# OpenPPL/ppq

Hardware: AMD Instinct MI355X
Metric: calibration samples/sec (RuntimeCalibrationPass, KL 2048-bin, ResNet-50 INT8) (higher is better)
Workload: dtype f32; 1 GPU; ResNet-50 topology (53 Conv + 1 Gemm, BN folded, seeded He init), RuntimeCalibrationPass kl 2048 bins, per-tensor INT8 activations, per-channel INT8 weights, 279 batches x 32 x 3x224x224 per GPU; samples=8928, batch=32, observed_tensors=72, rccl_ranks=1, async_observe=False, cache_params=False, channels_last=False, fuse_params=True, batch_observations=True, reuse_activations=False, replayed_batches=0, hip_graph=auto, graph_replays=0, miopen_find=False

## Files before the change

### include/ppq_hip.h

```cpp
#ifndef PPQ_HIP_H_
#define PPQ_HIP_H_

#include <stdint.h>

#ifdef __cplusplus
extern "C" {
#endif

typedef enum {
    PPQHIP_OK = 0,
    PPQHIP_ERR_INVALID_VALUE = -1,
    PPQHIP_ERR_UNSUPPORTED = -2,
    PPQHIP_ERR_HIP = -3
} ppqhip_status;

#define PPQHIP_ABI_VERSION 4

const char* ppqhip_last_error(void);
int ppqhip_version(void);
int ppqhip_device_arch(char* buf, int n);

int ppqhip_fq_linear_t(const float* x, const float* scale, const float* offset, float* out,
                       int64_t n, int clip_min, int clip_max, int rounding, void* stream);

int ppqhip_fq_linear_c(const float* x, const float* scale, const float* offset, float* out,
                       int64_t n, int64_t num_channel, int64_t elem_per_channel,
                       int clip_min, int clip_max, int rounding, void* stream);

int ppqhip_to_int_t(const float* x, const float* scale, const float* offset, void* out, int64_t n,
                    int clip_min, int clip_max, int rounding, int out_dtype, void* stream);
int ppqhip_to_int_c(const float* x, const float* scale, const float* offset, void* out, int64_t n,
                    int64_t num_channel, int64_t elem_per_channel, int clip_min, int clip_max,
                    int rounding, int out_dtype, void* stream);

typedef struct ppqhip_fq_job {
    const float* x;
    const float* scale;
    const float* offset;
    float* out;
    int64_t n, num_channel, elem_per_channel;
    int32_t clip_min, clip_max;
} ppqhip_fq_job;
int64_t ppqhip_fq_linear_multi_table_bytes(int num_jobs);
int ppqhip_fq_linear_multi(const ppqhip_fq_job* jobs, int num_jobs, int rounding, void* device_table,
                           int upload, void* stream);

int ppqhip_fq_linear_t_bwd(const float* x, const float* scale, const float* offset,
                           const float* grad_y, float* grad_x, float* grad_s, int64_t n,
                           int clip_min, int clip_max, int rounding, void* stream);

int ppqhip_fq_linear_c_bwd(const float* x, const float* scale, const float* offset,
                           const float* grad_y, float* grad_x, float* grad_s, int64_t n,
                           int64_t num_channel, int64_t elem_per_channel,
                           int clip_min, int clip_max, int rounding, void* stream);

int64_t ppqhip_fq_linear_t_bwd_partials(int64_t n);
int ppqhip_fq_linear_t_bwd_main(const float* x, const float* scale, const float* offset, const float* grad_y, float* grad_x,
                                float* partial, int64_t n, int clip_min, int clip_max, int rounding, void* stream);
typedef struct ppqhip_lsq_finish_job {
    const float* partial;
    float* grad_s;
    int64_t n;
    int32_t clip_min, clip_max;
} ppqhip_lsq_finish_job;
int ppqhip_lsq_finish_multi(const ppqhip_lsq_finish_job* jobs, int num_jobs, void* stream);

typedef struct ppqhip_lsq_job {
    const float* x;
    const float* scale;
    const float* offset;
    const float* grad_y;
    float* grad_x;
    float* grad_s;
    int64_t n, num_channel, elem_per_channel;
    int32_t clip_min, clip_max;
} ppqhip_lsq_job;
int ppqhip_fq_linear_c_bwd_multi(const ppqhip_lsq_job* jobs, int num_jobs, int rounding, void* stream);

int ppqhip_fq_float_t(const float* x, const float* scale, const float* offset, float* out,
                      int64_t n, int exponent, int mantissa, float clip_min, float clip_max,
                      int rounding, void* stream);

int ppqhip_fq_float_c(const float* x, const float* scale, const float* offset, float* out,
                      int64_t n, int64_t num_channel, int64_t elem_per_channel,
                      int exponent, int mantissa, float clip_min, float clip_max,
                      int rounding, void* stream);

typedef struct ppqhip_float_search_job {
    const float* x;
    int64_t rows, row_len;
    int32_t exponent, mantissa;
    float clip_min, clip_max;
} ppqhip_float_search_job;
int64_t ppqhip_float_scale_search_table_bytes(int num_jobs);
int ppqhip_float_scale_search(const ppqhip_float_search_job* jobs, int num_jobs, const float* candidates,
                              int num_candidates, int rounding, void* device_table, double* out, void* stream);

typedef struct ppqhip_fq_float_job {
    const float* x;
    const float* scale;
    const float* offset;
    float* out;
    int64_t n, num_channel, elem_per_channel;
    int32_t exponent, mantissa;
    float clip_min, clip_max;
} ppqhip_fq_float_job;
int64_t ppqhip_fq_float_multi_table_bytes(int num_jobs);
int ppqhip_fq_float_multi(const ppqhip_fq_float_job* jobs, int num_jobs, int rounding, void* device_table,
                          int upload, void* stream);

int ppqhip_fq_float_c_bwd(const float* x, const float* scale, const float* offset,
                          const float* grad_y, float* grad_x, float* grad_s, int64_t n,
                          int64_t num_channel, int64_t elem_per_channel,
                          int exponent, int mantissa, float clip_min, float clip_max,
                          int rounding, void* stream);

int64_t ppqhip_hist_workspace_bytes(int64_t n, int64_t num_bins);
int ppqhip_hist_sym_t(const float* x, int64_t n, float hist_scale, int clip_outliers,
                      int32_t* hist, int64_t num_bins, void* workspace, void* stream);

int ppqhip_hist_asym_t(const float* x, int64_t n, float min_value, float max_value,
                       int clip_outliers, int32_t* hist, int64_t num_bins, void* workspace,
                       void* stream);

int ppqhip_hist_sym_c(const float* x, int64_t n, int64_t num_channel, int64_t elem_per_channel,
                      float hist_scale, int clip_outliers, int32_t* hist, int64_t num_bins,
                      void* stream);

int ppqhip_hist_sym_c_scales(const float* x, int64_t n, int64_t num_channel, int64_t elem_per_channel,
                             const float* hist_scales, int clip_outliers, int32_t* hist,
                             int64_t num_bins, void* stream);
int ppqhip_hist_asym_c_ranges(const float* x, int64_t n, int64_t num_channel, int64_t elem_per_channel,
                              const float* mins, const float* maxs, int clip_outliers, int32_t* hist,
                              int64_t num_bins, void* stream);

int64_t ppqhip_quantile_workspace_bytes(int64_t n);
int ppqhip_quantile_t(const float* x, int64_t n, float q, float* dest, uint32_t* hint, void* workspace,
                      void* stream);

typedef struct ppqhip_quantile_job {
    const float* x;
    float* dest;
    uint32_t* hint;
    int64_t n;
} ppqhip_quantile_job;
int64_t ppqhip_quantile_multi_workspace_bytes(int num_jobs, int64_t total_elems);
int ppqhip_quantile_t_multi(const ppqhip_quantile_job* jobs, int num_jobs, float q, void* workspace,
                            void* stream);
void ppqhip_quantile_debug_layout(int64_t* out);
void ppqhip_quantile_hot_layout(int64_t* out);

int ppqhip_isotone_t(const float* x, int64_t n, float* dest, void* workspace, void* stream);

int64_t ppqhip_minmax_workspace_bytes(int64_t n);
int ppqhip_minmax_t(const float* x, int64_t n, float* minmax, void* workspace, void* stream);

int ppqhip_minmax_c(const float* x, int64_t n, int64_t num_channel, int64_t elem_per_channel,
                    float* mins, float* maxs, void* stream);

typedef struct ppqhip_minmax_c_job {
    const float* x;
    float* mins;
    float* maxs;
    int64_t n, num_channel, elem_per_channel;
    int32_t fresh, reserved;
} ppqhip_minmax_c_job;
int ppqhip_minmax_c_multi(const ppqhip_minmax_c_job* jobs, int num_jobs, void* stream);

int ppqhip_channel_sum(const float* x, int64_t n, int64_t num_channel, int64_t elem_per_channel,
                       double* sums, void* stream);

int64_t ppqhip_hist_rows(void);
int ppqhip_hist_sym_t_rows(const float* x, int64_t n, float hist_scale, int clip_outliers,
                           int32_t* rows, int64_t num_bins, void* stream);
int ppqhip_hist_asym_t_rows(const float* x, int64_t n, float min_value, float max_value,
                            int clip_outliers, int32_t* rows, int64_t num_bins, void* stream);
typedef struct ppqhip_minmax_job {
    const float* x;
    float* slots;
    int64_t n;
} ppqhip_minmax_job;
int ppqhip_minmax_t_slots_multi(const ppqhip_minmax_job* jobs, int num_jobs, void* stream);

typedef struct ppqhip_hist_job {
    const float* x;
    int32_t* rows;
    int64_t n;
    float p0, p1;
} ppqhip_hist_job;
int ppqhip_hist_t_rows_multi(const ppqhip_hist_job* jobs, int num_jobs, int asymmetric,
                             int clip_outliers, int64_t num_bins, void* stream);
int ppqhip_hist_rows_finish(const int32_t* rows, int64_t num_bins, int32_t* hist, void* stream);
int ppqhip_check_bin_rule(const float* x, int64_t n, float min_value, float hist_scale, int asymmetric, uint64_t* out, void* stream);
int64_t ppqhip_minmax_slots(void);
int ppqhip_minmax_t_slots(const float* x, int64_t n, float* slots, void* stream);
int ppqhip_minmax_slots_finish(const float* slots, float* minmax, void* stream);

float ppqhip_mse_loss_host(const int64_t* hist, int64_t num_bins, int start, int step, int end);

int64_t ppqhip_mse_search_workspace_bytes(int64_t num_hist);
int ppqhip_mse_search(const int32_t* hist, int64_t num_hist, int64_t num_bins,
                      const double* hist_scale, const double* min_value,
                      int quant_min, int quant_max, int symmetrical, int32_t* best,
                      void* workspace, void* stream);

int64_t ppqhip_kl_num_candidates(int64_t num_bins, int num_of_bits);
int ppqhip_kl_losses(const int32_t* hist, int64_t num_hist, int64_t num_bins, int num_of_bits,
                     double* losses, void* stream);

int ppqhip_tensor_clip_t(const float* value, const float* reference, const float* limit,
                         float* out, int64_t n, void* stream);
int ppqhip_tensor_clip_c(const float* value, const float* reference, const float* limit,
                         float* out, int64_t n, int64_t num_channel, int64_t elem_per_channel,
                         void* stream);
int ppqhip_rounding_loss(const float* x, const float* scale, const float* offset, float* out,
                         int64_t n, int64_t num_channel, int64_t elem_per_channel,
                         int clip_min, int clip_max, int rounding, void* stream);
int ppqhip_rounding_loss_bwd(const float* x, const float* dy, const float* scale,
                             const float* offset, float* dx, int64_t n, int64_t num_channel,
                             int64_t elem_per_channel, int clip_min, int clip_max, int rounding,
                             void* stream);

int ppqhip_bias_act(float* y, const float* bias, int64_t n, int64_t num_channel, int64_t elem_per_channel,
                    int relu, void* stream);
int ppqhip_bias_add_act(float* a, const float* bias_a, float* b, const float* bias_b, float* out,
                        int64_t n, int64_t num_channel, int64_t elem_per_channel, int relu, void* stream);

typedef struct ppqhip_adaround_job {
    const float* w;
    const float* v;
    const float* scale;
    const float* offset;
    float* out;
    const float* dy;
    int64_t n, num_channel, elem_per_channel;
    int32_t qmin, qmax;
} ppqhip_adaround_job;
int ppqhip_adaround_fwd_multi(const ppqhip_adaround_job* jobs, int num_jobs, void* stream);
int ppqhip_adaround_bwd_multi(const ppqhip_adaround_job* jobs, int num_jobs, const float* reg, void* stream);

typedef struct ppqhip_roundtune_job {
    const float* w;
    const float* r;
    const float* scale;
    const float* offset;
    float* out;
    int64_t n, num_channel, elem_per_channel;
    int32_t qmin, qmax;
} ppqhip_roundtune_job;
int ppqhip_roundtune_fwd_multi(const ppqhip_roundtune_job* jobs, int num_jobs, void* stream);

typedef struct ppqhip_fetch_rows_job {
    const float* x;
    const int32_t* index;
    float* out;
    int64_t rows, row_len, count;
} ppqhip_fetch_rows_job;
int ppqhip_fetch_rows_multi(const ppqhip_fetch_rows_job* jobs, int num_jobs, void* stream);
typedef struct ppqhip_measure_rows_job {
    const float* p;
    const float* r;
    const int32_t* index;
    double* sums;
    int64_t rows, row_len, count;
} ppqhip_measure_rows_job;
int ppqhip_measure_rows_multi(const ppqhip_measure_rows_job* jobs, int num_jobs, void* stream);
enum { PPQHIP_MEASURE_SNR = 0, PPQHIP_MEASURE_MSE = 1, PPQHIP_MEASURE_COSINE = 2 };
enum { PPQHIP_REDUCE_MEAN = 0, PPQHIP_REDUCE_MAX = 1 };
typedef struct ppqhip_measure_finish_job {
    const double* sums;
    double* acc;
    float* row_out;
    int64_t rows, count;
    int32_t method, reduce;
} ppqhip_measure_finish_job;
int ppqhip_measure_finish_multi(const ppqhip_measure_finish_job* jobs, int num_jobs, void* stream);

typedef struct ppqhip_equalize_segment {
    const float* base;
    int64_t extent;
    int64_t div, a, b;
    int64_t outer, stride, run;
    float multiplier;
    int32_t downstream;
} ppqhip_equalize_segment;
typedef struct ppqhip_equalize_scale_job {
    const ppqhip_equalize_segment* segments;
    float* scale;
    int32_t num_segments, num_channel;
    float value_threshold;
    int32_t reserved;
} ppqhip_equalize_scale_job;
int ppqhip_equalize_scale_multi(const ppqhip_equalize_scale_job* jobs, int num_jobs, void* stream);
typedef struct ppqhip_equalize_apply_job {
    float* x;
    const float* scale;
    int64_t n, run, inner, group_out;
    int64_t num_scale;
    int32_t divide, reserved;
} ppqhip_equalize_apply_job;
int ppqhip_equalize_apply_multi(const ppqhip_equalize_apply_job* jobs, int num_jobs, void* stream);

typedef struct ppqhip_split_plan_job {
    const ppqhip_equalize_segment* segments;
    int32_t* src_of;
    int32_t* count;
    int32_t num_segments, num_channel;
    float value_threshold;
    int32_t reserved;
} ppqhip_split_plan_job;
int ppqhip_split_plan_multi(const ppqhip_split_plan_job* jobs, int num_jobs, void* stream);
typedef struct ppqhip_split_apply_job {
    const float* x;
    float* out;
    const int32_t* src_of;
    int64_t n, run;
    int32_t num_channel, count;
} ppqhip_split_apply_job;
int ppqhip_split_apply_multi(const ppqhip_split_apply_job* jobs, int num_jobs, void* stream);

typedef struct ppqhip_ssd_scales_job {
    ppqhip_equalize_segment first, last;
    const float* act_range;
    float* scales;
    float* ranges;
    int32_t num_channel;
    float channel_ratio;
} ppqhip_ssd_scales_job;
int ppqhip_ssd_scales_multi(const ppqhip_ssd_scales_job* jobs, int num_jobs, void* stream);
typedef struct ppqhip_ssd_apply_job {
    const float* x;
    float* out;
    const float* scales;
    int64_t n, run, inner, group_out;
    int64_t num_channel;
    int32_t divide, reserved;
} ppqhip_ssd_apply_job;
int ppqhip_ssd_apply_multi(const ppqhip_ssd_apply_job* jobs, int num_jobs, void* stream);
typedef struct ppqhip_fq_measure_rows_job {
    const float* y;
    const float* r;
    const float* scale;
    const float* offset;
    double* sums;
    int64_t rows, count;
    int64_t num_channel, elem_per_channel;
    int32_t clip_min, clip_max, rounding, reserved;
} ppqhip_fq_measure_rows_job;
int ppqhip_fq_measure_rows_multi(const ppqhip_fq_measure_rows_job* jobs, int num_jobs, void* stream);

typedef struct ppqhip_stat_job {
    const float* p;
    const float* r;
    float* rec;
    int64_t n;
    int32_t bins, reserved;
} ppqhip_stat_job;
int ppqhip_stat_moments_multi(const ppqhip_stat_job* jobs, int num_jobs, void* stream);
int ppqhip_stat_shape_multi(const ppqhip_stat_job* jobs, int num_jobs, void* stream);

enum { PPQHIP_MXFP8_E4M3 = 0, PPQHIP_MXFP8_E5M2 = 1, PPQHIP_MXFP6_E3M2 = 2, PPQHIP_MXFP6_E2M3 = 3, PPQHIP_MXFP4_E2M1 = 4,
       PPQHIP_MXINT8 = 5 };
int ppqhip_mx_fq(const float* x, float* y, uint8_t* scale_codes, int64_t outer, int64_t axis_len, int64_t inner, int format,
                 void* stream);
typedef struct ppqhip_mx_job {
    const float* x;
    float* y;
    uint8_t* scale_codes;
    int64_t outer, axis_len, inner;
    int32_t format, reserved;
} ppqhip_mx_job;
int ppqhip_mx_fq_multi(const ppqhip_mx_job* jobs, int num_jobs, void* stream);

int ppqhip_mx_pack(const float* x, uint8_t* elements, uint8_t* scales, int64_t outer, int64_t axis_len, int64_t inner, int format,
                   void* stream);
typedef struct ppqhip_mx_pack_job {
    const float* x;
    uint8_t* elements;
    uint8_t* scales;
    int64_t outer, axis_len, inner;
    int32_t format, reserved;
} ppqhip_mx_pack_job;
int ppqhip_mx_pack_multi(const ppqhip_mx_pack_job* jobs, int num_jobs, void* stream);
int ppqhip_mx_unpack(const uint8_t* elements, const uint8_t* scales, float* y, int64_t outer, int64_t axis_len, int64_t inner,
                     int format, void* stream);
typedef struct ppqhip_mx_unpack_job {
    const uint8_t* elements;
    const uint8_t* scales;
    float* y;
    int64_t outer, axis_len, inner;
    int32_t format, reserved;
} ppqhip_mx_unpack_job;
int ppqhip_mx_unpack_multi(const ppqhip_mx_unpack_job* jobs, int num_jobs, void* stream);

int ppqhip_mx_gemm(const uint8_t* a_elements, const uint8_t* a_scales, int a_format, const uint8_t* b_elements,
                   const uint8_t* b_scales, int b_format, const float* bias, float* c, int64_t m, int64_t n, int64_t k,
                   void* stream);

int ppqhip_mx_conv2d(const uint8_t* x_elements, const uint8_t* x_scales, int x_format, const uint8_t* w_elements,
                     const uint8_t* w_scales, int w_format, const float* bias, float* y, int64_t n, int64_t c, int64_t h, int64_t w,
                     int64_t o, int64_t kh, int64_t kw, int64_t stride_h, int64_t stride_w, int64_t pad_h, int64_t pad_w,
                     int64_t dil_h, int64_t dil_w, void* stream);

#define PPQHIP_PROF_MAX_KERNELS 48
typedef struct {
    char name[48];
    int64_t launches;
    double total_ms;
    double total_bytes;
} ppqhip_prof_entry;
int ppqhip_prof_enable(int on);
int ppqhip_prof_collect(ppqhip_prof_entry* entries, int max_entries);
double ppqhip_prof_event_overhead_us(void* stream, int pairs);

#ifdef __cplusplus
}
#endif
#endif
```

### ppq_amd/_lib.py

```python
import ctypes
import os

_HERE = os.path.dirname(os.path.abspath(__file__))
LIB_PATH = os.path.join(_HERE, 'libppq_hip.so')

c_f32p = ctypes.c_void_p
c_i32p = ctypes.c_void_p
c_f64p = ctypes.c_void_p
c_i64 = ctypes.c_int64
c_int = ctypes.c_int
c_flt = ctypes.c_float
c_vp = ctypes.c_void_p

ABI_VERSION = 4


class ProfEntry(ctypes.Structure):
    _fields_ = [('name', ctypes.c_char * 48), ('launches', ctypes.c_int64),
                ('total_ms', ctypes.c_double), ('total_bytes', ctypes.c_double)]


PROTOTYPES = {
    'ppqhip_last_error': (ctypes.c_char_p, []),
    'ppqhip_version': (c_int, []),
    'ppqhip_device_arch': (c_int, [ctypes.c_char_p, c_int]),
    'ppqhip_fq_linear_t': (c_int, [c_f32p, c_f32p, c_f32p, c_f32p, c_i64, c_int, c_int, c_int, c_vp]),
    'ppqhip_fq_linear_c': (c_int, [c_f32p, c_f32p, c_f32p, c_f32p, c_i64, c_i64, c_i64, c_int, c_int, c_int, c_vp]),
    'ppqhip_to_int_t': (c_int, [c_f32p, c_f32p, c_f32p, c_vp, c_i64, c_int, c_int, c_int, c_int, c_vp]),
    'ppqhip_to_int_c': (c_int, [c_f32p, c_f32p, c_f32p, c_vp, c_i64, c_i64, c_i64, c_int, c_int, c_int, c_int, c_vp]),
    'ppqhip_fq_linear_t_bwd': (c_int, [c_f32p, c_f32p, c_f32p, c_f32p, c_f32p, c_f32p, c_i64, c_int, c_int, c_int,
                                       c_vp]),
    'ppqhip_fq_linear_c_bwd': (c_int, [c_f32p, c_f32p, c_f32p, c_f32p, c_f32p, c_f32p, c_i64, c_i64, c_i64, c_int,
                                       c_int, c_int, c_vp]),
    'ppqhip_fq_linear_c_bwd_multi': (c_int, [c_vp, c_int, c_int, c_vp]),
    'ppqhip_fq_linear_t_bwd_partials': (c_i64, [c_i64]),
    'ppqhip_fq_linear_t_bwd_main': (c_int, [c_f32p, c_f32p, c_f32p, c_f32p, c_f32p, c_f32p, c_i64, c_int, c_int, c_int, c_vp]),
    'ppqhip_lsq_finish_multi': (c_int, [c_vp, c_int, c_vp]),
    'ppqhip_bias_act': (c_int, [c_f32p, c_f32p, c_i64, c_i64, c_i64, c_int, c_vp]),
    'ppqhip_bias_add_act': (c_int, [c_f32p, c_f32p, c_f32p, c_f32p, c_f32p, c_i64, c_i64, c_i64, c_int, c_vp]),
    'ppqhip_fq_float_t': (c_int, [c_f32p, c_f32p, c_f32p, c_f32p, c_i64, c_int, c_int, c_flt, c_flt, c_int, c_vp]),
    'ppqhip_fq_float_c': (c_int, [c_f32p, c_f32p, c_f32p, c_f32p, c_i64, c_i64, c_i64, c_int, c_int, c_flt, c_flt,
                                  c_int, c_vp]),
    'ppqhip_fq_float_c_bwd': (c_int, [c_f32p, c_f32p, c_f32p, c_f32p, c_f32p, c_f32p, c_i64, c_i64, c_i64, c_int,
                                      c_int, c_flt, c_flt, c_int, c_vp]),
    'ppqhip_hist_workspace_bytes': (c_i64, [c_i64, c_i64]),
    'ppqhip_hist_sym_t': (c_int, [c_f32p, c_i64, c_flt, c_int, c_i32p, c_i64, c_vp, c_vp]),
    'ppqhip_hist_asym_t': (c_int, [c_f32p, c_i64, c_flt, c_flt, c_int, c_i32p, c_i64, c_vp, c_vp]),
    'ppqhip_hist_sym_c': (c_int, [c_f32p, c_i64, c_i64, c_i64, c_flt, c_int, c_i32p, c_i64, c_vp]),
    'ppqhip_hist_sym_c_scales': (c_int, [c_f32p, c_i64, c_i64, c_i64, c_f32p, c_int, c_i32p, c_i64, c_vp]),
    'ppqhip_hist_asym_c_ranges': (c_int, [c_f32p, c_i64, c_i64, c_i64, c_f32p, c_f32p, c_int, c_i32p, c_i64, c_vp]),
    'ppqhip_quantile_workspace_bytes': (c_i64, [c_i64]),
    'ppqhip_quantile_t': (c_int, [c_f32p, c_i64, c_flt, c_f32p, c_vp, c_vp, c_vp]),
    'ppqhip_isotone_t': (c_int, [c_f32p, c_i64, c_f32p, c_vp, c_vp]),
    'ppqhip_minmax_workspace_bytes': (c_i64, [c_i64]),
    'ppqhip_minmax_t': (c_int, [c_f32p, c_i64, c_f32p, c_vp, c_vp]),
    'ppqhip_minmax_c': (c_int, [c_f32p, c_i64, c_i64, c_i64, c_f32p, c_f32p, c_vp]),
    'ppqhip_minmax_c_multi': (c_int, [c_vp, c_int, c_vp]),
    'ppqhip_fq_linear_multi_table_bytes': (c_i64, [c_int]),
    'ppqhip_fq_linear_multi': (c_int, [c_vp, c_int, c_int, c_vp, c_int, c_vp]),
    'ppqhip_float_scale_search_table_bytes': (c_i64, [c_int]),
    'ppqhip_float_scale_search': (c_int, [c_vp, c_int, c_vp, c_int, c_int, c_vp, c_vp, c_vp]),
    'ppqhip_fq_float_multi_table_bytes': (c_i64, [c_int]),
    'ppqhip_fq_float_multi': (c_int, [c_vp, c_int, c_int, c_vp, c_int, c_vp]),
    'ppqhip_quantile_multi_workspace_bytes': (c_i64, [c_int, c_i64]),
    'ppqhip_quantile_t_multi': (c_int, [c_vp, c_int, c_flt, c_vp, c_vp]),
    'ppqhip_quantile_debug_layout': (None, [c_vp]),
    'ppqhip_quantile_hot_layout': (None, [c_vp]),
    'ppqhip_minmax_t_slots_multi': (c_int, [c_vp, c_int, c_vp]),
    'ppqhip_hist_t_rows_multi': (c_int, [c_vp, c_int, c_int, c_int, c_i64, c_vp]),
    'ppqhip_channel_sum': (c_int, [c_f32p, c_i64, c_i64, c_i64, c_f64p, c_vp]),
    'ppqhip_hist_rows': (c_i64, []),
    'ppqhip_hist_sym_t_rows': (c_int, [c_f32p, c_i64, c_flt, c_int, c_i32p, c_i64, c_vp]),
    'ppqhip_hist_asym_t_rows': (c_int, [c_f32p, c_i64, c_flt, c_flt, c_int, c_i32p, c_i64, c_vp]),
    'ppqhip_hist_rows_finish': (c_int, [c_i32p, c_i64, c_i32p, c_vp]),
    'ppqhip_check_bin_rule': (c_int, [c_f32p, c_i64, c_flt, c_flt, c_int, c_vp, c_vp]),
    'ppqhip_minmax_slots': (c_i64, []),
    'ppqhip_minmax_t_slots': (c_int, [c_f32p, c_i64, c_f32p, c_vp]),
    'ppqhip_minmax_slots_finish': (c_int, [c_f32p, c_f32p, c_vp]),
    'ppqhip_mse_loss_host': (c_flt, [ctypes.POINTER(ctypes.c_int64), c_i64, c_int, c_int, c_int]),
    'ppqhip_mse_search_workspace_bytes': (c_i64, [c_i64]),
    'ppqhip_mse_search': (c_int, [c_i32p, c_i64, c_i64, c_f64p, c_f64p, c_int, c_int, c_int, c_i32p, c_vp, c_vp]),
    'ppqhip_kl_num_candidates': (c_i64, [c_i64, c_int]),
    'ppqhip_kl_losses': (c_int, [c_i32p, c_i64, c_i64, c_int, c_f64p, c_vp]),
    'ppqhip_tensor_clip_t': (c_int, [c_f32p, c_f32p, c_f32p, c_f32p, c_i64, c_vp]),
    'ppqhip_tensor_clip_c': (c_int, [c_f32p, c_f32p, c_f32p, c_f32p, c_i64, c_i64, c_i64, c_vp]),
    'ppqhip_rounding_loss': (c_int, [c_f32p, c_f32p, c_f32p, c_f32p, c_i64, c_i64, c_i64, c_int, c_int, c_int, c_vp]),
    'ppqhip_rounding_loss_bwd': (c_int, [c_f32p, c_f32p, c_f32p, c_f32p, c_f32p, c_i64, c_i64, c_i64, c_int, c_int,
                                         c_int, c_vp]),
    'ppqhip_adaround_fwd_multi': (c_int, [c_vp, c_int, c_vp]),
    'ppqhip_adaround_bwd_multi': (c_int, [c_vp, c_int, c_f32p, c_vp]),
    'ppqhip_roundtune_fwd_multi': (c_int, [c_vp, c_int, c_vp]),
    'ppqhip_equalize_scale_multi': (c_int, [c_vp, c_int, c_vp]),
    'ppqhip_equalize_apply_multi': (c_int, [c_vp, c_int, c_vp]),
    'ppqhip_split_plan_multi': (c_int, [c_vp, c_int, c_vp]),
    'ppqhip_split_apply_multi': (c_int, [c_vp, c_int, c_vp]),
    'ppqhip_ssd_scales_multi': (c_int, [c_vp, c_int, c_vp]),
    'ppqhip_ssd_apply_multi': (c_int, [c_vp, c_int, c_vp]),
    'ppqhip_fq_measure_rows_multi': (c_int, [c_vp, c_int, c_vp]),
    'ppqhip_fetch_rows_multi': (c_int, [c_vp, c_int, c_vp]),
    'ppqhip_measure_rows_multi': (c_int, [c_vp, c_int, c_vp]),
    'ppqhip_measure_finish_multi': (c_int, [c_vp, c_int, c_vp]),
    'ppqhip_stat_moments_multi': (c_int, [c_vp, c_int, c_vp]),
    'ppqhip_stat_shape_multi': (c_int, [c_vp, c_int, c_vp]),
    'ppqhip_mx_fq': (c_int, [c_f32p, c_f32p, c_vp, c_i64, c_i64, c_i64, c_int, c_vp]),
    'ppqhip_mx_fq_multi': (c_int, [c_vp, c_int, c_vp]),
    'ppqhip_mx_pack': (c_int, [c_f32p, c_vp, c_vp, c_i64, c_i64, c_i64, c_int, c_vp]),
    'ppqhip_mx_pack_multi': (c_int, [c_vp, c_int, c_vp]),
    'ppqhip_mx_unpack': (c_int, [c_vp, c_vp, c_f32p, c_i64, c_i64, c_i64, c_int, c_vp]),
    'ppqhip_mx_unpack_multi': (c_int, [c_vp, c_int, c_vp]),
    'ppqhip_mx_gemm': (c_int, [c_vp, c_vp, c_int, c_vp, c_vp, c_int, c_f32p, c_f32p, c_i64, c_i64, c_i64, c_vp]),
    'ppqhip_prof_enable': (c_int, [c_int]),
    'ppqhip_mx_conv2d': (c_int, [c_vp, c_vp, c_int, c_vp, c_vp, c_int, c_f32p, c_f32p] + [c_i64] * 13 + [c_vp]),
    'ppqhip_prof_collect': (c_int, [ctypes.POINTER(ProfEntry), c_int]),
    'ppqhip_prof_event_overhead_us': (ctypes.c_double, [c_vp, c_int]),
}

if not os.path.exists(LIB_PATH):
    raise ImportError(
        f'{LIB_PATH} is missing: the HIP kernel library has not been built.  Run '
        '`python -c "import __graft_entry__ as g; g.build()"` or `make -C ppq_amd/csrc` (needs hipcc, '
        'targets gfx950).  ppq_amd has no CPU / PyTorch fallback by design.')

import torch

_torch_hip = os.path.join(os.path.dirname(torch.__file__), 'lib', 'libamdhip64.so')
if os.path.exists(_torch_hip):
    ctypes.CDLL(_torch_hip, mode=ctypes.RTLD_GLOBAL)

try:
    lib = ctypes.CDLL(LIB_PATH)
except OSError as e:
    raise ImportError(f'cannot load {LIB_PATH}: {e}') from e

for _name, (_res, _args) in PROTOTYPES.items():
    _fn = getattr(lib, _name)
    _fn.restype = _res
    _fn.argtypes = _args


if lib.ppqhip_version() != ABI_VERSION:
    raise ImportError(f'{LIB_PATH} has ABI version {lib.ppqhip_version()}, this package needs {ABI_VERSION}: rebuild it '
                      '(`make -C ppq_amd/csrc` or `python -c "import __graft_entry__ as g; g.build()"`)')


def last_error() -> str:
    msg = lib.ppqhip_last_error()
    return msg.decode('utf-8', 'replace') if msg else ''
```

### ppq_amd/csrc/epilogue.hip

```cpp
#include "common.hpp"

namespace ppqhip {
namespace {

constexpr int kEpTileU = 2;
constexpr int kEpSmallU = 1;
constexpr long long kEpSmallElems = 1ll << 20;

struct EpArgs {
    float* a;
    const float* bias_a;
    float* b;
    const float* bias_b;
    float* out;
    uint32_t nvec;
    uint32_t tail;
    int ntail;
    FastDiv epc;
    FastDiv nc;
};

__device__ __forceinline__ uint32_t channel_of(uint32_t i, const FastDiv& epc, const FastDiv& nc) {
    const uint32_t row = fdiv(i, epc);
    return row - fdiv(row, nc) * nc.d;
}

__device__ __forceinline__ float act(float v, bool relu) {
    return (relu && !__builtin_isnan(v)) ? __builtin_fmaxf(v, 0.f) : v;
}

__device__ __forceinline__ float4 add4(const float4& x, const float4& y) {
    return make_float4(x.x + y.x, x.y + y.y, x.z + y.z, x.w + y.w);
}

template <bool RELU>
__device__ __forceinline__ float4 act4(const float4& v) {
    return make_float4(act(v.x, RELU), act(v.y, RELU), act(v.z, RELU), act(v.w, RELU));
}

template <bool PLANE>
__device__ __forceinline__ float4 bias4(const float* __restrict__ bias, uint32_t v, const FastDiv& epc, const FastDiv& nc) {
    if (PLANE) {
        const float t = bias[channel_of(v, epc, nc)];
        return make_float4(t, t, t, t);
    }
    const uint32_t i = v * 4u;
    return make_float4(bias[channel_of(i, epc, nc)], bias[channel_of(i + 1, epc, nc)], bias[channel_of(i + 2, epc, nc)],
                       bias[channel_of(i + 3, epc, nc)]);
}

template <bool RESID, bool BIAS_B, bool RELU>
__device__ __forceinline__ void epilogue_elem(const EpArgs& p, uint32_t i, const FastDiv& epc) {
    const uint32_t c = channel_of(i, epc, p.nc);
    const float x = p.a[i] + p.bias_a[c];
    if (!RESID) { p.a[i] = act(x, RELU); return; }
    p.a[i] = x;
    float y = p.b[i];
    if (BIAS_B) { y = y + p.bias_b[c]; p.b[i] = y; }
    p.out[i] = act(x + y, RELU);
}

template <int U, bool RESID, bool BIAS_B, bool RELU, bool PLANE>
__global__ __launch_bounds__(kBlock) void epilogue_kernel(EpArgs p) {
    const uint32_t base = blockIdx.x * (kBlock * U) + threadIdx.x;
    float4* a4 = reinterpret_cast<float4*>(p.a);
    float4* b4 = reinterpret_cast<float4*>(p.b);
    float4* o4 = reinterpret_cast<float4*>(p.out);
    float4 a[U], ba[U], b[U], bb[U];
#pragma unroll
    for (int k = 0; k < U; k++) {
        const uint32_t vv = min(base + k * kBlock, p.nvec - 1);
        a[k] = a4[vv];
        ba[k] = bias4<PLANE>(p.bias_a, vv, p.epc, p.nc);
        if (RESID) b[k] = b4[vv];
        if (BIAS_B) bb[k] = bias4<PLANE>(p.bias_b, vv, p.epc, p.nc);
    }
#pragma unroll
    for (int k = 0; k < U; k++) {
        const uint32_t vv = base + k * kBlock;
        if (vv >= p.nvec) continue;
        const float4 x = add4(a[k], ba[k]);
        if (!RESID) { a4[vv] = act4<RELU>(x); continue; }
        a4[vv] = x;
        float4 y = b[k];
        if (BIAS_B) { y = add4(y, bb[k]); b4[vv] = y; }
        o4[vv] = act4<RELU>(add4(x, y));
    }
    if (!PLANE && blockIdx.x == 0 && (int)threadIdx.x < p.ntail)
        epilogue_elem<RESID, BIAS_B, RELU>(p, p.tail + threadIdx.x, p.epc);
}

template <bool RESID, bool BIAS_B, bool RELU>
__global__ __launch_bounds__(kBlock) void epilogue_scalar_kernel(EpArgs p) {
    const uint32_t stride = gridDim.x * kBlock;
    for (uint32_t i = blockIdx.x * kBlock + threadIdx.x; i < (uint32_t)p.ntail; i += stride)
        epilogue_elem<RESID, BIAS_B, RELU>(p, i, p.epc);
}

template <bool RESID, bool BIAS_B, bool RELU>
void launch_epilogue(EpArgs p, int64_t n, int64_t C, int64_t epc, bool aligned, hipStream_t st) {
    p.nc = make_fastdiv((uint32_t)C);
    if (!aligned || n < 4) {
        p.nvec = 0; p.tail = 0; p.ntail = (int)n;
        p.epc = make_fastdiv((uint32_t)epc);
        hipLaunchKernelGGL((epilogue_scalar_kernel<RESID, BIAS_B, RELU>), dim3(stream_grid(n, kBlock)), dim3(kBlock), 0, st, p);
        return;
    }
    p.nvec = (uint32_t)(n >> 2);
    p.tail = p.nvec * 4u;
    p.ntail = (int)(n & 3);
    const bool plane = (epc % 4 == 0);
    p.epc = make_fastdiv((uint32_t)(plane ? epc / 4 : epc));
#define PPQ_LAUNCH_EP(U, PLANE)                                                                                          \
    hipLaunchKernelGGL((epilogue_kernel<U, RESID, BIAS_B, RELU, PLANE>), dim3((p.nvec + kBlock * U - 1) / (kBlock * U)),   \
                       dim3(kBlock), 0, st, p)
    if (n <= kEpSmallElems) {
        if (plane) PPQ_LAUNCH_EP(kEpSmallU, true); else PPQ_LAUNCH_EP(kEpSmallU, false);
    } else {
        if (plane) PPQ_LAUNCH_EP(kEpTileU, true); else PPQ_LAUNCH_EP(kEpTileU, false);
    }
#undef PPQ_LAUNCH_EP
}

int validate(int64_t n, int64_t C, int64_t epc, const char* what) {
    if (n <= 0 || n > 0x7fffffffLL) {
        set_error("%s: n=%lld is empty or has more than 2^31 - 1 elements", what, (long long)n);
        return PPQHIP_ERR_INVALID_VALUE;
    }
    if (C <= 0 || epc <= 0 || C > 0x7fffffffLL || epc > 0x7fffffffLL || n % (C * epc) != 0) {
        set_error("%s: n=%lld is not [outer, %lld channels, %lld elem/channel]", what, (long long)n, (long long)C,
                  (long long)epc);
        return PPQHIP_ERR_INVALID_VALUE;
    }
    return PPQHIP_OK;
}

}
}

using namespace ppqhip;

extern "C" {

int ppqhip_bias_act(float* y, const float* bias, int64_t n, int64_t num_channel, int64_t elem_per_channel, int relu,
                    void* stream) {
    if (int st = validate(n, num_channel, elem_per_channel, "bias_act")) return st;
    if (!y || !bias) { set_error("bias_act: null pointer"); return PPQHIP_ERR_INVALID_VALUE; }
    hipStream_t s = (hipStream_t)stream;
    EpArgs p{};
    p.a = y; p.bias_a = bias;
    const bool aligned = aligned16(y);
    if (relu) launch_epilogue<false, false, true>(p, n, num_channel, elem_per_channel, aligned, s);
    else launch_epilogue<false, false, false>(p, n, num_channel, elem_per_channel, aligned, s);
    return finish_launch("bias_act");
}

int ppqhip_bias_add_act(float* a, const float* bias_a, float* b, const float* bias_b, float* out, int64_t n,
                        int64_t num_channel, int64_t elem_per_channel, int relu, void* stream) {
    if (int st = validate(n, num_channel, elem_per_channel, "bias_add_act")) return st;
    if (!a || !bias_a || !b || !out) { set_error("bias_add_act: null pointer"); return PPQHIP_ERR_INVALID_VALUE; }
    hipStream_t s = (hipStream_t)stream;
    EpArgs p{};
    p.a = a; p.bias_a = bias_a; p.b = b; p.bias_b = bias_b; p.out = out;
    const bool aligned = aligned16(a) && aligned16(b) && aligned16(out);
    if (bias_b) {
        if (relu) launch_epilogue<true, true, true>(p, n, num_channel, elem_per_channel, aligned, s);
        else launch_epilogue<true, true, false>(p, n, num_channel, elem_per_channel, aligned, s);
    } else {
        if (relu) launch_epilogue<true, false, true>(p, n, num_channel, elem_per_channel, aligned, s);
        else launch_epilogue<true, false, false>(p, n, num_channel, elem_per_channel, aligned, s);
    }
    return finish_launch("bias_add_act");
}

}
```

### ppq_amd/csrc/reduce.hip

```cpp
#include <cmath>
#include <cstdlib>
#include <vector>

#include "common.hpp"

namespace ppqhip {

__device__ __forceinline__ void block_minmax_commit(float mn, float mx, float* gmin, float* gmax, float* lds) {
    mn = wave_min(mn);
    mx = wave_max(mx);
    const int wid = threadIdx.x >> 6, lane = threadIdx.x & 63, nw = blockDim.x >> 6;
    if (lane == 0) { lds[wid] = mn; lds[8 + wid] = mx; }
    __syncthreads();
    if (threadIdx.x == 0) {
        for (int w = 1; w < nw; w++) { mn = fminf(mn, lds[w]); mx = fmaxf(mx, lds[8 + w]); }
        if (mn <= mx) {
            atomic_min_f32(gmin, mn);
            atomic_max_f32(gmax, mx);
        }
    }
}

template <int U, bool NT>
__global__ __launch_bounds__(kBlock) void minmax_t_kernel(const float* __restrict__ x, uint32_t n, int vec_ok,
                                                          float* __restrict__ minmax, float* __restrict__ partial,
                                                          int accumulate) {
    __shared__ float lds[16];
    float mn = INFINITY, mx = -INFINITY;
    stream_elems<U, NT>(x, n, vec_ok != 0, [&](float a) { mn = fminf(mn, a); mx = fmaxf(mx, a); });
    if (partial == nullptr) { block_minmax_commit(mn, mx, &minmax[0], &minmax[1], lds); return; }
    mn = wave_min(mn);
    mx = wave_max(mx);
    const int wid = threadIdx.x >> 6, lane = threadIdx.x & 63;
    if (lane == 0) { lds[wid] = mn; lds[8 + wid] = mx; }
    __syncthreads();
    if (threadIdx.x == 0) {
        for (int w = 1; w < kBlock / kWave; w++) { mn = fminf(mn, lds[w]); mx = fmaxf(mx, lds[8 + w]); }
        if (accumulate) {
            mn = fminf(mn, partial[2 * blockIdx.x]);
            mx = fmaxf(mx, partial[2 * blockIdx.x + 1]);
        }
        partial[2 * blockIdx.x] = mn;
        partial[2 * blockIdx.x + 1] = mx;
    }
}

constexpr int kMinMaxMultiMax = 96;
constexpr int kMMBlock = 256, kMMU = 2;
constexpr int kMMWgPerCu = 8;
constexpr int kMMGrid = kNumCU * kMMWgPerCu;
constexpr uint32_t kMMTileVec = (uint32_t)kMMBlock * kMMU, kMMTileElems = kMMTileVec * 4;
static_assert(kMMGrid <= kNumCU * 8, "one slot per workgroup");
struct MinMaxJob {
    const float* x;
    float* slots;
    uint32_t n;
    uint32_t first_tile;
};
struct MinMaxJobs {
    MinMaxJob job[kMinMaxMultiMax];
    uint32_t count;
    uint32_t total_tiles;
};
__host__ __device__ inline uint32_t mm_job_tiles(uint32_t n, bool vec_ok) {
    if (!vec_ok) return (n + kMMTileElems - 1) / kMMTileElems;
    const uint32_t full = (n >> 2) / kMMTileVec;
    return full + (n > full * kMMTileElems ? 1u : 0u);
}

template <bool NT>
__global__ __launch_bounds__(kMMBlock) void minmax_persistent_kernel(const MinMaxJobs jobs) {
    __shared__ float lds[32];
    const uint32_t G = gridDim.x, g = blockIdx.x;
    uint32_t t, t_end;
    even_split(jobs.total_tiles, G, g, t, t_end);
    if (t >= t_end) return;
    uint32_t lo = 0, hi = jobs.count;
    while (hi - lo > 1) {
        const uint32_t mid = (lo + hi) >> 1;
        if (jobs.job[mid].first_tile <= t) lo = mid; else hi = mid;
    }
    for (uint32_t j = lo; t < t_end; j++) {
        const MinMaxJob& job = jobs.job[j];
        const uint32_t j_end = (j + 1 < jobs.count) ? jobs.job[j + 1].first_tile : jobs.total_tiles;
        uint32_t k = t - job.first_tile;
        const uint32_t k1 = min(t_end, j_end) - job.first_tile;
        t = min(t_end, j_end);
        const float* __restrict__ x = job.x;
        const uint32_t n = job.n;
        const bool vec_ok = (reinterpret_cast<uintptr_t>(x) & 15u) == 0;
        const uint32_t full = vec_ok ? (n >> 2) / kMMTileVec : 0u;
        const uint32_t kf = min(k1, full);
        float mn = INFINITY, mx = -INFINITY;
        if (k < kf) {
            const float4* xv = reinterpret_cast<const float4*>(x) + threadIdx.x;
            float4 bufa[kMMU], bufb[kMMU];
            auto fetch = [&](float4 (&buf)[kMMU], uint32_t tile) {
                const float4* p = xv + (size_t)tile * kMMTileVec;
#pragma unroll
                for (int u = 0; u < kMMU; u++) buf[u] = load4<NT>(p + u * kMMBlock);
            };
            auto consume = [&](const float4 (&buf)[kMMU]) {
#pragma unroll
                for (int u = 0; u < kMMU; u++) {
                    mn = fminf(fminf(mn, buf[u].x), fminf(buf[u].y, fminf(buf[u].z, buf[u].w)));
                    mx = fmaxf(fmaxf(mx, buf[u].x), fmaxf(buf[u].y, fmaxf(buf[u].z, buf[u].w)));
                }
            };
            fetch(bufa, k);
            for (;;) {
                fetch(bufb, min(k + 1, kf - 1));
                consume(bufa);
                if (++k >= kf) break;
                fetch(bufa, min(k + 1, kf - 1));
                consume(bufb);
                if (++k >= kf) break;
            }
        }
        for (; k < k1; k++) {
            const uint32_t e0 = k * kMMTileElems + threadIdx.x;
#pragma unroll 4
            for (int r = 0; r < 4 * kMMU; r++) {
                const uint32_t i = e0 + r * kMMBlock;
                if (i < n) { const float a = x[i]; mn = fminf(mn, a); mx = fmaxf(mx, a); }
            }
        }
        mn = wave_min(mn);
        mx = wave_max(mx);
        const int wid = threadIdx.x >> 6, lane = threadIdx.x & 63;
        if (lane == 0) { lds[wid] = mn; lds[16 + wid] = mx; }
        __syncthreads();
        if (threadIdx.x == 0) {
            for (int w = 1; w < kMMBlock / kWave; w++) { mn = fminf(mn, lds[w]); mx = fmaxf(mx, lds[16 + w]); }
            job.slots[2 * g] = fminf(mn, job.slots[2 * g]);
            job.slots[2 * g + 1] = fmaxf(mx, job.slots[2 * g + 1]);
        }
        __syncthreads();
    }
}

template <int K, bool PING = false, bool NT = false>
__global__ __launch_bounds__(kMMBlock) void minmax_small_kernel(const float* __restrict__ x, uint32_t n, float* __restrict__ slots) {
    __shared__ float lds[32];
    const uint32_t G = gridDim.x, g = blockIdx.x;
    float s_mn = INFINITY, s_mx = -INFINITY;
    if (threadIdx.x == 0) { s_mn = slots[2 * g]; s_mx = slots[2 * g + 1]; }
    const uint32_t nvec = n >> 2, full_rows = nvec / kMMBlock;
    uint32_t r0, r1;
    even_split(full_rows, G, g, r0, r1);
    const float4* xv = reinterpret_cast<const float4*>(x) + threadIdx.x;
    float mn = INFINITY, mx = -INFINITY;
    auto fetch = [&](float4 (&buf)[K], uint32_t r) {
#pragma unroll
        for (int k = 0; k < K; k++) buf[k] = load4<NT>(xv + (size_t)min(r + (uint32_t)k, r1 - 1) * kMMBlock);
    };
    auto fold = [&](const float4 (&buf)[K]) {
#pragma unroll
        for (int k = 0; k < K; k++) {
            mn = fminf(fminf(mn, buf[k].x), fminf(buf[k].y, fminf(buf[k].z, buf[k].w)));
            mx = fmaxf(fmaxf(mx, buf[k].x), fmaxf(buf[k].y, fmaxf(buf[k].z, buf[k].w)));
        }
    };
    if (PING) {
        if (r0 < r1) {
            float4 bufa[K], bufb[K];
            uint32_t r = r0;
            fetch(bufa, r);
            for (;;) {
                fetch(bufb, r + K);
                fold(bufa);
                r += K;
                if (r >= r1) break;
                fetch(bufa, r + K);
                fold(bufb);
                r += K;
                if (r >= r1) break;
            }
        }
    } else {
        for (uint32_t r = r0; r < r1; r += K) {
            float4 buf[K];
            fetch(buf, r);
            fold(buf);
        }
    }
    if (g == G - 1) {
        for (uint32_t i = full_rows * kMMBlock * 4 + threadIdx.x; i < n; i += kMMBlock) { const float a = x[i]; mn = fminf(mn, a); mx = fmaxf(mx, a); }
    }
    mn = wave_min(mn);
    mx = wave_max(mx);
    const int wid = threadIdx.x >> 6, lane = threadIdx.x & 63;
    if (lane == 0) { lds[wid] = mn; lds[16 + wid] = mx; }
    __syncthreads();
    if (threadIdx.x == 0) {
        for (int w = 1; w < kMMBlock / kWave; w++) { mn = fminf(mn, lds[w]); mx = fmaxf(mx, lds[16 + w]); }
        slots[2 * g] = fminf(mn, s_mn);
        slots[2 * g + 1] = fmaxf(mx, s_mx);
    }
}

__global__ __launch_bounds__(kBlock) void minmax_finish_kernel(const float* __restrict__ partial, uint32_t count,
                                                               float* __restrict__ minmax) {
    __shared__ float lds[16];
    float mn = INFINITY, mx = -INFINITY;
    for (uint32_t i = threadIdx.x; i < count; i += kBlock) {
        mn = fminf(mn, partial[2 * i]);
        mx = fmaxf(mx, partial[2 * i + 1]);
    }
    mn = wave_min(mn);
    mx = wave_max(mx);
    const int wid = threadIdx.x >> 6, lane = threadIdx.x & 63;
    if (lane == 0) { lds[wid] = mn; lds[8 + wid] = mx; }
    __syncthreads();
    if (threadIdx.x == 0) {
        for (int w = 1; w < kBlock / kWave; w++) { mn = fminf(mn, lds[w]); mx = fmaxf(mx, lds[8 + w]); }
        minmax[0] = fminf(minmax[0], mn);
        minmax[1] = fmaxf(minmax[1], mx);
    }
}

constexpr int kMMCU = 16;
constexpr int kMMCWavesPerCu = 16;
constexpr uint32_t kMMCChunk = 8192;
__global__ __launch_bounds__(kBlock) void minmax_c_wave_kernel(const float* __restrict__ x, uint32_t epc, int vec_ok, uint32_t C,
                                                               uint32_t outer, uint32_t K, uint32_t chunks, uint32_t items,
                                                               float* __restrict__ mins, float* __restrict__ maxs) {
    const uint32_t item = blockIdx.x * (kBlock / kWave) + (threadIdx.x >> 6);
    if (item >= items) return;
    const uint32_t lane = threadIdx.x & 63;
    const uint32_t rc = item / chunks, chunk = item - rc * chunks;
    const uint32_t g = rc / C, c = rc - g * C;
    const uint32_t n0 = g * K, n1 = min(n0 + K, outer);
    const uint32_t lo = chunk * kMMCChunk, hi = min(lo + kMMCChunk, epc);
    float mn = INFINITY, mx = -INFINITY;
    for (uint32_t n = n0; n < n1; n++) {
        const float* xr = x + ((size_t)n * C + c) * epc;
        if (vec_ok) {
            const float4* xv = reinterpret_cast<const float4*>(xr);
            const uint32_t v1 = hi >> 2;
            for (uint32_t v0 = (lo >> 2) + lane; v0 < v1; v0 += 64 * kMMCU) {
                float4 a[kMMCU];
#pragma unroll
                for (int u = 0; u < kMMCU; u++) a[u] = xv[min(v0 + 64 * u, v1 - 1)];
#pragma unroll
                for (int u = 0; u < kMMCU; u++) {
                    mn = fminf(fminf(mn, a[u].x), fminf(a[u].y, fminf(a[u].z, a[u].w)));
                    mx = fmaxf(fmaxf(mx, a[u].x), fmaxf(a[u].y, fmaxf(a[u].z, a[u].w)));
                }
            }
        } else {
            for (uint32_t j = lo + lane; j < hi; j += 64) { const float a = xr[j]; mn = fminf(mn, a); mx = fmaxf(mx, a); }
        }
    }
    mn = wave_min(mn);
    mx = wave_max(mx);
    if (lane == 0 && mn <= mx) { atomic_min_f32(&mins[c], mn); atomic_max_f32(&maxs[c], mx); }
}

__global__ __launch_bounds__(kBlock) void minmax_c_generic_kernel(const float* __restrict__ x, uint32_t n,
                                                                  FastDiv elem_per_channel, FastDiv num_channel,
                                                                  int use_lds, float* __restrict__ mins,
                                                                  float* __restrict__ maxs) {
    extern __shared__ float mm[];
    const uint32_t C = num_channel.d;
    if (use_lds) {
        for (uint32_t c = threadIdx.x; c < C; c += kBlock) { mm[c] = INFINITY; mm[C + c] = -INFINITY; }
        __syncthreads();
    }
    const uint32_t stride = gridDim.x * kBlock;
    for (uint32_t i = blockIdx.x * kBlock + threadIdx.x; i < n; i += stride) {
        const float a = x[i];
        if (a != a) continue;
        const uint32_t row = fdiv(i, elem_per_channel);
        const uint32_t c = row - fdiv(row, num_channel) * C;
        if (use_lds) { atomic_min_f32(&mm[c], a); atomic_max_f32(&mm[C + c], a); }
        else { atomic_min_f32(&mins[c], a); atomic_max_f32(&maxs[c], a); }
    }
    if (use_lds) {
        __syncthreads();
        for (uint32_t c = threadIdx.x; c < C; c += kBlock) {
            if (mm[c] <= mm[C + c]) { atomic_min_f32(&mins[c], mm[c]); atomic_max_f32(&maxs[c], mm[C + c]); }
        }
    }
}

__device__ __forceinline__ double wave_sum_f64(double v) {
#pragma unroll
    for (int m = 32; m > 0; m >>= 1) v += __shfl_xor(v, m, 64);
    return v;
}

__global__ __launch_bounds__(kBlock) void channel_sum_row_kernel(const float* __restrict__ x, uint32_t rows_per_channel,
                                                                 uint32_t C, uint32_t epc, int vec_ok,
                                                                 double* __restrict__ partial) {
    __shared__ double lds[kBlock / kWave];
    const uint32_t c = blockIdx.x, s = blockIdx.y, S = gridDim.y;
    double acc = 0.0;
    for (uint32_t n = s; n < rows_per_channel; n += S) {
        const float* xr = x + ((size_t)n * C + c) * epc;
        if (vec_ok) {
            const float4* xv = reinterpret_cast<const float4*>(xr);
            const uint32_t v1 = epc >> 2;
            for (uint32_t v = threadIdx.x; v < v1; v += 4 * kBlock) {
                float4 a[4];
#pragma unroll
                for (int u = 0; u < 4; u++) a[u] = xv[min(v + u * kBlock, v1 - 1)];
#pragma unroll
                for (int u = 0; u < 4; u++)
                    if (v + u * kBlock < v1) acc += ((double)a[u].x + (double)a[u].y) + ((double)a[u].z + (double)a[u].w);
            }
        } else {
            for (uint32_t j = threadIdx.x; j < epc; j += kBlock) acc += (double)xr[j];
        }
    }
    acc = wave_sum_f64(acc);
    const int wid = threadIdx.x >> 6, lane = threadIdx.x & 63;
    if (lane == 0) lds[wid] = acc;
    __syncthreads();
    if (threadIdx.x == 0) {
        double t = lds[0];
        for (int w = 1; w < kBlock / kWave; w++) t += lds[w];
        partial[(size_t)s * C + c] = t;
    }
}

__global__ __launch_bounds__(kBlock) void channel_sum_single_kernel(const float* __restrict__ x, uint32_t rows_per_channel, uint32_t C,
                                                                    uint32_t epc, double* __restrict__ sums) {
    __shared__ double lds[kBlock / kWave];
    const uint32_t c = blockIdx.x;
    const uint32_t v1 = epc >> 2;
    double acc = 0.0;
    const double seed = threadIdx.x == 0 ? sums[c] : 0.0;
    for (uint32_t n = 0; n < rows_per_channel; n += 2) {
        const float4* x0 = reinterpret_cast<const float4*>(x + ((size_t)n * C + c) * epc);
        const float4* x1 = reinterpret_cast<const float4*>(x + ((size_t)min(n + 1, rows_per_channel - 1) * C + c) * epc);
        const bool two = n + 1 < rows_per_channel;
        for (uint32_t v = threadIdx.x; v < v1; v += 4 * kBlock) {
            float4 a[4], b[4];
#pragma unroll
            for (int u = 0; u < 4; u++) { a[u] = x0[min(v + u * kBlock, v1 - 1)]; b[u] = x1[min(v + u * kBlock, v1 - 1)]; }
#pragma unroll
            for (int u = 0; u < 4; u++)
                if (v + u * kBlock < v1) acc += ((double)a[u].x + (double)a[u].y) + ((double)a[u].z + (double)a[u].w);
            if (two) {
#pragma unroll
                for (int u = 0; u < 4; u++)
                    if (v + u * kBlock < v1) acc += ((double)b[u].x + (double)b[u].y) + ((double)b[u].z + (double)b[u].w);
            }
        }
    }
    acc = wave_sum_f64(acc);
    const int wid = threadIdx.x >> 6, lane = threadIdx.x & 63;
    if (lane == 0) lds[wid] = acc;
    __syncthreads();
    if (threadIdx.x == 0) {
        double t = lds[0];
        for (int w = 1; w < kBlock / kWave; w++) t += lds[w];
        sums[c] = seed + t;
    }
}

__global__ __launch_bounds__(kBlock) void channel_sum_finish_kernel(const double* __restrict__ partial, uint32_t S,
                                                                    uint32_t C, double* __restrict__ sums) {
    const uint32_t c = blockIdx.x * kBlock + threadIdx.x;
    if (c >= C) return;
    double t = 0.0;
    for (uint32_t s = 0; s < S; s++) t += partial[(size_t)s * C + c];
    sums[c] += t;
}

__global__ __launch_bounds__(kBlock) void channel_sum_generic_kernel(const float* __restrict__ x, uint32_t outer,
                                                                     uint32_t C, uint32_t epc,
                                                                     double* __restrict__ sums) {
    const uint32_t c = blockIdx.x * kBlock + threadIdx.x;
    if (c >= C) return;
    double t = 0.0;
    for (uint32_t n = 0; n < outer; n++) {
        const float* xr = x + ((size_t)n * C + c) * epc;
        for (uint32_t j = 0; j < epc; j++) t += (double)xr[j];
    }
    sums[c] += t;
}

__device__ __forceinline__ bool aligned16_dev(const void* p) { return (reinterpret_cast<uintptr_t>(p) & 15u) == 0; }

struct Top2 { float a1, a2, b1, b2; };

__device__ __forceinline__ void top2_push(Top2& t, float v) {
    if (v > t.a1) { t.a2 = t.a1; t.a1 = v; } else if (v > t.a2) t.a2 = v;
    if (v < t.b1) { t.b2 = t.b1; t.b1 = v; } else if (v < t.b2) t.b2 = v;
}
__device__ __forceinline__ void top2_merge(Top2& t, const Top2& o) {
    const float hi = fmaxf(t.a1, o.a1);
    const float second = fmaxf(fminf(t.a1, o.a1), fmaxf(t.a2, o.a2));
    t.a1 = hi; t.a2 = second;
    const float lo = fminf(t.b1, o.b1);
    const float second_lo = fminf(fmaxf(t.b1, o.b1), fminf(t.b2, o.b2));
    t.b1 = lo; t.b2 = second_lo;
}
__device__ __forceinline__ Top2 top2_wave(Top2 t) {
#pragma unroll
    for (int m = 32; m > 0; m >>= 1) {
        Top2 o;
        o.a1 = __shfl_xor(t.a1, m, 64); o.a2 = __shfl_xor(t.a2, m, 64);
        o.b1 = __shfl_xor(t.b1, m, 64); o.b2 = __shfl_xor(t.b2, m, 64);
        top2_merge(t, o);
    }
    return t;
}

__global__ __launch_bounds__(kBlock) void isotone_kernel(const float* __restrict__ x, uint32_t n,
                                                         const Top2* __restrict__ partial_in, uint32_t n_partial,
                                                         Top2* __restrict__ partial_out, float* __restrict__ dest,
                                                         uint32_t n_total) {
    __shared__ Top2 lds[kBlock / kWave];
    Top2 t{-INFINITY, -INFINITY, INFINITY, INFINITY};
    if (partial_in == nullptr) {
        stream_elems<4>(x, n, aligned16_dev(x), [&](float v) { top2_push(t, v); });
    } else {
        for (uint32_t i = threadIdx.x; i < n_partial; i += kBlock) top2_merge(t, partial_in[i]);
    }
    t = top2_wave(t);
    const int wid = threadIdx.x >> 6, lane = threadIdx.x & 63;
    if (lane == 0) lds[wid] = t;
    __syncthreads();
    if (threadIdx.x == 0) {
        for (int w = 1; w < kBlock / kWave; w++) top2_merge(t, lds[w]);
        if (dest == nullptr) partial_out[blockIdx.x] = t;
        else if (n_total == 1) { dest[0] = dest[1] = dest[2] = dest[3] = t.a1; }
        else { dest[0] = t.a1; dest[1] = t.a2; dest[2] = t.b1; dest[3] = t.b2; }
    }
}

constexpr int kIsotoneBlocks = 1024;
static_assert(kIsotoneBlocks * sizeof(Top2) <= 65536, "the partials must fit ppqhip_quantile_workspace_bytes (quantile.hip: >= 74 KB)");

static int validate(int64_t n, const char* what) {
    if (n <= 0) { set_error("%s: tensor is empty", what); return PPQHIP_ERR_INVALID_VALUE; }
    if (n > 0x7fffffffLL) { set_error("%s: too many elements", what); return PPQHIP_ERR_INVALID_VALUE; }
    return PPQHIP_OK;
}

constexpr int kMMCMultiMax = 64;
struct MMCJob {
    const float* x;
    float* mins;
    float* maxs;
    uint32_t C, epc, outer, chunks;
    uint32_t vec_ok, fresh;
};
struct MMCMultiArgs {
    MMCJob jobs[kMMCMultiMax];
    uint32_t first_item[kMMCMultiMax];
    uint32_t count;
    uint32_t items;
};
static_assert(sizeof(MMCMultiArgs) <= 4096, "kernel arguments are limited to 4 KB");

__global__ __launch_bounds__(kBlock) void minmax_c_multi_kernel(const MMCMultiArgs args) {
    const uint32_t item = blockIdx.x * (kBlock / kWave) + (threadIdx.x >> 6);
    if (item >= args.items) return;
    const uint32_t lane = threadIdx.x & 63;
    uint32_t lo = 0, hi = args.count;
    while (hi - lo > 1) {
        const uint32_t mid = (lo + hi) >> 1;
        if (args.first_item[mid] <= item) lo = mid; else hi = mid;
    }
    const MMCJob& j = args.jobs[__builtin_amdgcn_readfirstlane(lo)];
    const uint32_t local = item - args.first_item[lo];
    const uint32_t row = local / j.chunks, chunk = local - row * j.chunks;
    const uint32_t c = row % j.C;
    const uint32_t e0 = chunk * kMMCChunk, e1 = min(e0 + kMMCChunk, j.epc);
    const float* xr = j.x + (size_t)row * j.epc;
    float mn = INFINITY, mx = -INFINITY;
    if (j.vec_ok) {
        const float4* xv = reinterpret_cast<const float4*>(xr);
        const uint32_t v1 = e1 >> 2;
        constexpr int U = 8;
        for (uint32_t v0 = (e0 >> 2) + lane; v0 < v1; v0 += 64 * U) {
            float4 a[U];
#pragma unroll
            for (int u = 0; u < U; u++) a[u] = xv[min(v0 + 64 * u, v1 - 1)];
#pragma unroll
            for (int u = 0; u < U; u++) {
                mn = fminf(fminf(mn, a[u].x), fminf(a[u].y, fminf(a[u].z, a[u].w)));
                mx = fmaxf(fmaxf(mx, a[u].x), fmaxf(a[u].y, fmaxf(a[u].z, a[u].w)));
            }
        }
    } else {
        for (uint32_t e = e0 + lane; e < e1; e += 64) { const float a = xr[e]; mn = fminf(mn, a); mx = fmaxf(mx, a); }
    }
    mn = wave_min(mn);
    mx = wave_max(mx);
    if (lane == 0) {
        if (j.fresh) { j.mins[c] = mn; j.maxs[c] = mx; }
        else if (mn <= mx) { atomic_min_f32(&j.mins[c], mn); atomic_max_f32(&j.maxs[c], mx); }
    }
}

}

using namespace ppqhip;

extern "C" {

int64_t ppqhip_minmax_workspace_bytes(int64_t n) { (void)n; return (int64_t)sizeof(float) * 2 * kNumCU * 8; }

static int minmax_t_impl(const float* x, int64_t n, float* minmax, void* workspace, float* slots, void* stream) {
    if (int st = validate(n, "minmax_t")) return st;
    hipStream_t s = (hipStream_t)stream;
    LaunchScope scope(K_MINMAX_T, 4.0 * (double)n, s);
    const bool nt = n >= (48ll << 20);
    const int grid = stream_grid(n, kBlock * 4 * 4, num_cu() * 8);
    float* partial = slots;
    const int accumulate = slots != nullptr;
    if (!slots && grid > 32) {
        partial = workspace ? (float*)workspace : (float*)scratch(s, sizeof(float) * 2 * (size_t)grid);
        if (partial == nullptr) return PPQHIP_ERR_HIP;
    }
    if (nt)
        hipLaunchKernelGGL((minmax_t_kernel<4, true>), dim3(grid), dim3(kBlock), 0, s, x, (uint32_t)n,
// ... 229 lines not shown
```

### ppq_amd/ffi.py

```python
import math
import threading
import weakref
from typing import List

import numpy as np
import torch

from . import _lib
from ._lib import lib

_KERNEL_FAILURE = 'Kernel Failure, '


_raw_stream = torch._C._cuda_getCurrentRawStream
_get_device = torch._C._cuda_getDevice


def _stream() -> int:
    return _raw_stream(_get_device())


def _check(t: torch.Tensor, dtype: torch.dtype, name: str) -> None:
    if not isinstance(t, torch.Tensor):
        raise TypeError(f'{name}: expected a torch.Tensor, got {type(t)}')
    if t.dtype != dtype:
        raise RuntimeError(_KERNEL_FAILURE + 'Invalid dtype of Input tensor: ' + name)
    if t.numel() == 0:
        raise RuntimeError(_KERNEL_FAILURE + 'Tensor is empty: ' + name)
    if not t.is_cuda:
        raise RuntimeError(_KERNEL_FAILURE + f'{name} is not on the GPU (ppq_amd has no CPU path)')


_F32 = torch.float32


def _f32(t, name):
    try:
        if t.dtype is _F32 and t.is_cuda and t.numel() > 0: return
    except AttributeError:
        pass
    _check(t, torch.float32, name + '(Expect to be FP32)')


def _dense(t: torch.Tensor, channel_axis=None) -> torch.Tensor:
    if t.is_contiguous(): return t
    if channel_axis is None or channel_axis % t.dim() == 0:
        if t.dim() == 4 and t.is_contiguous(memory_format=torch.channels_last): return t
        if t.dim() == 5 and t.is_contiguous(memory_format=torch.channels_last_3d): return t
    return t.contiguous()


def _raise(status: int) -> None:
    if status != 0:
        raise RuntimeError(_KERNEL_FAILURE + _lib.last_error())


def _geometry(shape, channel_axis: int):
    ndim = len(shape)
    if channel_axis < 0: channel_axis += ndim
    if not 0 <= channel_axis < ndim:
        raise RuntimeError(_KERNEL_FAILURE + f'channel_axis {channel_axis} out of range for a {ndim}-d tensor')
    epc = 1
    for d in shape[channel_axis + 1:]:
        epc *= int(d)
    return int(shape[channel_axis]), epc


class _DeviceOf:
    __slots__ = ('idx', 'prev')

    def __init__(self, t: torch.Tensor):
        self.idx = t.device.index
        self.prev = None

    def __enter__(self):
        if self.idx is not None and self.idx != _get_device():
            self.prev = _get_device()
            torch.cuda.set_device(self.idx)

    def __exit__(self, *a):
        if self.prev is not None:
            torch.cuda.set_device(self.prev)


_workspaces = {}
_MAX_WORKSPACES = 16


def _workspace(device: torch.device, nbytes: int) -> torch.Tensor:
    key = (device.index, _stream())
    ws = _workspaces.pop(key, None)
    if ws is None or ws.numel() < nbytes:
        ws = torch.empty(max(nbytes, 1 << 16), dtype=torch.uint8, device=device)
    _workspaces[key] = ws
    while len(_workspaces) > _MAX_WORKSPACES:
        _workspaces.pop(next(iter(_workspaces)))
    return ws


_MINMAX_JOB = np.dtype([('x', '<u8'), ('slots', '<u8'), ('n', '<i8')])
_FQ_JOB = np.dtype([('x', '<u8'), ('scale', '<u8'), ('offset', '<u8'), ('out', '<u8'), ('n', '<i8'),
                    ('num_channel', '<i8'), ('elem_per_channel', '<i8'), ('clip_min', '<i4'), ('clip_max', '<i4')])
_FQ_FLOAT_JOB = np.dtype([('x', '<u8'), ('scale', '<u8'), ('offset', '<u8'), ('out', '<u8'), ('n', '<i8'),
                          ('num_channel', '<i8'), ('elem_per_channel', '<i8'), ('exponent', '<i4'), ('mantissa', '<i4'),
                          ('clip_min', '<f4'), ('clip_max', '<f4')])
_FLOAT_SEARCH_JOB = np.dtype([('x', '<u8'), ('rows', '<i8'), ('row_len', '<i8'), ('exponent', '<i4'), ('mantissa', '<i4'),
                              ('clip_min', '<f4'), ('clip_max', '<f4')])
_LSQ_JOB = np.dtype([('x', '<u8'), ('scale', '<u8'), ('offset', '<u8'), ('grad_y', '<u8'), ('grad_x', '<u8'), ('grad_s', '<u8'),
                     ('n', '<i8'), ('num_channel', '<i8'), ('elem_per_channel', '<i8'), ('clip_min', '<i4'), ('clip_max', '<i4')])
_LSQ_FINISH_JOB = np.dtype([('partial', '<u8'), ('grad_s', '<u8'), ('n', '<i8'), ('clip_min', '<i4'), ('clip_max', '<i4')])
_MINMAX_C_JOB = np.dtype([('x', '<u8'), ('mins', '<u8'), ('maxs', '<u8'), ('n', '<i8'), ('num_channel', '<i8'),
                          ('elem_per_channel', '<i8'), ('fresh', '<i4'), ('reserved', '<i4')])
_QUANTILE_JOB = np.dtype([('x', '<u8'), ('dest', '<u8'), ('hint', '<u8'), ('n', '<i8')])

_owner_hints = weakref.WeakKeyDictionary()
_hint_owner = threading.local()


def quantile_hint(device: torch.device) -> torch.Tensor:
    return torch.zeros(8, dtype=torch.int32, device=device)


class quantile_hint_owner:
    __slots__ = ('owner', 'prev')

    def __init__(self, owner):
        self.owner, self.prev = owner, None

    def __enter__(self):
        self.prev = getattr(_hint_owner, 'current', None)
        _hint_owner.current = self.owner
        return self

    def __exit__(self, *a):
        _hint_owner.current = self.prev


def _owner_quantile_hint(device: torch.device, numel: int, q: float):
    owner = getattr(_hint_owner, 'current', None)
    if owner is None: return None
    try: per = _owner_hints.setdefault(owner, {})
    except TypeError: return None
    key = (device.index, int(numel), float(q))
    h = per.get(key)
    if h is None: h = per[key] = quantile_hint(device)
    return h


_HIST_JOB = np.dtype([('x', '<u8'), ('rows', '<u8'), ('n', '<i8'), ('p0', '<f4'), ('p1', '<f4')])


def _epilogue_geometry(ts, bias_list):
    t0 = ts[0]
    if not isinstance(t0, torch.Tensor) or t0.dtype is not _F32 or not t0.is_cuda or t0.dim() != 4 or t0.numel() == 0:
        return None
    shape, strides, dev = t0.shape, t0.stride(), t0.device
    for t in ts[1:]:
        if not isinstance(t, torch.Tensor) or t.dtype is not _F32 or t.device != dev or t.shape != shape or t.stride() != strides:
            return None
    C = int(shape[1])
    for bias in bias_list:
        if (not isinstance(bias, torch.Tensor) or bias.dtype is not _F32 or bias.device != dev or bias.dim() != 1
                or bias.numel() != C or not bias.is_contiguous()):
            return None
    if t0.is_contiguous(): return C, int(shape[2]) * int(shape[3])
    if t0.is_contiguous(memory_format=torch.channels_last): return C, 1
    return None


def bias_act_(y: torch.Tensor, bias: torch.Tensor, relu: bool) -> bool:
    geo = _epilogue_geometry([y], [bias])
    if geo is None: return False
    with _DeviceOf(y):
        _raise(lib.ppqhip_bias_act(y.data_ptr(), bias.data_ptr(), y.numel(), geo[0], geo[1], 1 if relu else 0, _stream()))
    return True


def bias_add_act(a: torch.Tensor, bias_a: torch.Tensor, b: torch.Tensor, bias_b, relu: bool):
    geo = _epilogue_geometry([a, b], [bias_a] if bias_b is None else [bias_a, bias_b])
    if geo is None or a.data_ptr() == b.data_ptr(): return None
    out = torch.empty_like(a)
    with _DeviceOf(a):
        _raise(lib.ppqhip_bias_add_act(a.data_ptr(), bias_a.data_ptr(), b.data_ptr(), 0 if bias_b is None else bias_b.data_ptr(),
                                       out.data_ptr(), a.numel(), geo[0], geo[1], 1 if relu else 0, _stream()))
    return out


_ADAROUND_JOB = np.dtype([('w', '<u8'), ('v', '<u8'), ('scale', '<u8'), ('offset', '<u8'), ('out', '<u8'), ('dy', '<u8'),
                          ('n', '<i8'), ('num_channel', '<i8'), ('elem_per_channel', '<i8'), ('qmin', '<i4'), ('qmax', '<i4')])


def _adaround_table(items, outs, dys=None):
    n = len(items)
    if len(outs) != n or (dys is not None and len(dys) != n):
        raise RuntimeError(_KERNEL_FAILURE + 'AdaRound: argument lists differ in length')
    jobs = np.zeros(n, dtype=_ADAROUND_JOB)
    dev = items[0][0].device
    for k, (w, v, s, o, axis, qmin, qmax) in enumerate(items):
        ts = [('Value', w), ('Rounding', v), ('Scale', s), ('Offset', o), ('Out', outs[k])] + ([('Dy', dys[k])] if dys is not None else [])
        for name, t in ts:
            _f32(t, name)
            if t.device != dev: raise RuntimeError(_KERNEL_FAILURE + f'AdaRound: item {k}: {name} is on another device')
            if not t.is_contiguous(): raise RuntimeError(_KERNEL_FAILURE + f'AdaRound: item {k}: {name} is not contiguous')
        for name, t in ts[1:2] + ts[4:]:
            if t.shape != w.shape: raise RuntimeError(_KERNEL_FAILURE + f'AdaRound: item {k}: {name} is not shaped like the weight')
        C, epc = _geometry(w.shape, axis) if axis is not None else (1, w.numel())
        if s.numel() != C or o.numel() != C:
            raise RuntimeError(_KERNEL_FAILURE + f'AdaRound: item {k}: scale / offset need {C} elements')
        jobs[k] = (w.data_ptr(), v.data_ptr(), s.data_ptr(), o.data_ptr(), outs[k].data_ptr(),
                   dys[k].data_ptr() if dys is not None else 0, w.numel(), C, epc, int(qmin), int(qmax))
    return jobs


def adaround_forward_multi(items, outs=None) -> List[torch.Tensor]:
    if not items: return []
    if outs is None: outs = [torch.empty_like(it[0]) for it in items]
    jobs = _adaround_table(items, outs)
    with _DeviceOf(items[0][0]):
        _raise(lib.ppqhip_adaround_fwd_multi(jobs.ctypes.data, len(items), _stream()))
    return outs


def adaround_backward_multi(items, dys, reg: torch.Tensor, dvs=None) -> List[torch.Tensor]:
    if not items: return []
    _f32(reg, 'Reg')
    if reg.numel() != 3 or not reg.is_contiguous() or reg.device != items[0][0].device:
        raise RuntimeError(_KERNEL_FAILURE + 'AdaRound: reg must be a contiguous float32[3] on the weights\' device')
    if dvs is None: dvs = [torch.empty_like(it[0]) for it in items]
    jobs = _adaround_table(items, dvs, dys)
    with _DeviceOf(items[0][0]):
        _raise(lib.ppqhip_adaround_bwd_multi(jobs.ctypes.data, len(items), reg.data_ptr(), _stream()))
    return dvs


_ROUNDTUNE_JOB = np.dtype([('w', '<u8'), ('r', '<u8'), ('scale', '<u8'), ('offset', '<u8'), ('out', '<u8'),
                           ('n', '<i8'), ('num_channel', '<i8'), ('elem_per_channel', '<i8'), ('qmin', '<i4'), ('qmax', '<i4')])


def _roundtune_table(items, outs):
    n = len(items)
    if len(outs) != n: raise RuntimeError(_KERNEL_FAILURE + 'RoundTuning: argument lists differ in length')
    jobs = np.zeros(n, dtype=_ROUNDTUNE_JOB)
    dev = items[0][0].device
    for k, (w, r, s, o, axis, qmin, qmax) in enumerate(items):
        ts = [('Value', w), ('Rounding', r), ('Scale', s), ('Offset', o), ('Out', outs[k])]
        for name, t in ts:
            _f32(t, name)
            if t.device != dev: raise RuntimeError(_KERNEL_FAILURE + f'RoundTuning: item {k}: {name} is on another device')
            if not t.is_contiguous(): raise RuntimeError(_KERNEL_FAILURE + f'RoundTuning: item {k}: {name} is not contiguous')
        for name, t in ts[1:2] + ts[4:]:
            if t.shape != w.shape: raise RuntimeError(_KERNEL_FAILURE + f'RoundTuning: item {k}: {name} is not shaped like the weight')
        C, epc = _geometry(w.shape, axis) if axis is not None else (1, w.numel())
        if s.numel() != C or o.numel() != C:
            raise RuntimeError(_KERNEL_FAILURE + f'RoundTuning: item {k}: scale / offset need {C} elements')
        jobs[k] = (w.data_ptr(), r.data_ptr(), s.data_ptr(), o.data_ptr(), outs[k].data_ptr(), w.numel(), C, epc, int(qmin), int(qmax))
    return jobs


def roundtune_forward_multi(items, outs=None) -> List[torch.Tensor]:
    if not items: return []
    if outs is None: outs = [torch.empty_like(it[0]) for it in items]
    jobs = _roundtune_table(items, outs)
    with _DeviceOf(items[0][0]):
        _raise(lib.ppqhip_roundtune_fwd_multi(jobs.ctypes.data, len(items), _stream()))
    return outs


_EQ_SEGMENT = np.dtype([('base', '<u8'), ('extent', '<i8'), ('div', '<i8'), ('a', '<i8'), ('b', '<i8'), ('outer', '<i8'),
                        ('stride', '<i8'), ('run', '<i8'), ('multiplier', '<f4'), ('downstream', '<i4')])
_EQ_SCALE_JOB = np.dtype([('segments', '<u8'), ('scale', '<u8'), ('num_segments', '<i4'), ('num_channel', '<i4'),
                          ('value_threshold', '<f4'), ('reserved', '<i4')])
_EQ_APPLY_JOB = np.dtype([('x', '<u8'), ('scale', '<u8'), ('n', '<i8'), ('run', '<i8'), ('inner', '<i8'), ('group_out', '<i8'),
                          ('num_scale', '<i8'), ('divide', '<i4'), ('reserved', '<i4')])


def _eq_tensor(t, what: str, k: int, dev):
    _f32(t, what)
    if t.device != dev: raise RuntimeError(_KERNEL_FAILURE + f'Equalization: item {k}: {what} is on another device')
    if not t.is_contiguous(): raise RuntimeError(_KERNEL_FAILURE + f'Equalization: item {k}: {what} is not contiguous')


def _segment_record(segment, k: int, dev, what: str = 'Value') -> tuple:
    t, div, a, b, outer, stride, run, mult, down = segment
    _eq_tensor(t, what, k, dev)
    return (t.data_ptr(), t.numel(), int(div), int(a), int(b), int(outer), int(stride), int(run), float(mult), 1 if down else 0)


class EqualizeTable:
    __slots__ = ('jobs', 'segments', 'keep', 'entry')

    def __init__(self, jobs, segments, keep, entry):
        self.jobs, self.segments, self.keep, self.entry = jobs, segments, keep, entry

    def __len__(self) -> int: return len(self.jobs)

    def run(self) -> None:
        if len(self.jobs) == 0: return
        with _DeviceOf(self.keep[0]):
            _raise(self.entry(self.jobs.ctypes.data, len(self.jobs), _stream()))


def equalize_scale_table(items) -> EqualizeTable:
    jobs = np.zeros(len(items), dtype=_EQ_SCALE_JOB)
    segs = np.zeros(sum(len(it[2]) for it in items), dtype=_EQ_SEGMENT)
    keep, records = [], []
    dev = items[0][0].device if items else None
    for k, (scale, threshold, segments) in enumerate(items):
        _eq_tensor(scale, 'Scale', k, dev)
        keep.append(scale)
        jobs[k] = (segs.ctypes.data + len(records) * _EQ_SEGMENT.itemsize, scale.data_ptr(), len(segments), scale.numel(), float(threshold), 0)
        for segment in segments:
            records.append(_segment_record(segment, k, dev))
            keep.append(segment[0])
    segs[:] = records
    return EqualizeTable(jobs, segs, keep, lib.ppqhip_equalize_scale_multi)


def equalize_apply_table(items) -> EqualizeTable:
    jobs = np.zeros(len(items), dtype=_EQ_APPLY_JOB)
    keep = []
    dev = items[0][0].device if items else None
    for k, (x, scale, run, inner, group_out, divide) in enumerate(items):
        _eq_tensor(x, 'Value', k, dev); _eq_tensor(scale, 'Scale', k, dev)
        keep += [x, scale]
        jobs[k] = (x.data_ptr(), scale.data_ptr(), x.numel(), int(run), int(inner), int(group_out), scale.numel(), 1 if divide else 0, 0)
    return EqualizeTable(jobs, None, keep, lib.ppqhip_equalize_apply_multi)


def equalize_scale_multi(items) -> None:
    (items if isinstance(items, EqualizeTable) else equalize_scale_table(items)).run()


def equalize_apply_multi(items) -> None:
    (items if isinstance(items, EqualizeTable) else equalize_apply_table(items)).run()


_SPLIT_PLAN_JOB = np.dtype([('segments', '<u8'), ('src_of', '<u8'), ('count', '<u8'), ('num_segments', '<i4'), ('num_channel', '<i4'),
                            ('value_threshold', '<f4'), ('reserved', '<i4')])
_SPLIT_APPLY_JOB = np.dtype([('x', '<u8'), ('out', '<u8'), ('src_of', '<u8'), ('n', '<i8'), ('run', '<i8'), ('num_channel', '<i4'),
                             ('count', '<i4')])
SPLIT_MAX_JOBS, SPLIT_MAX_SEGMENTS = 32, 72
SPLIT_BIT = -0x80000000


def _i32(t, what: str, k: int, dev, numel: int):
    if not (isinstance(t, torch.Tensor) and t.dtype == torch.int32 and t.is_contiguous() and t.numel() == numel):
        raise RuntimeError(_KERNEL_FAILURE + f'Channel split: item {k}: {what} must be a contiguous int32 tensor of {numel}')
    if not t.is_cuda: raise RuntimeError(_KERNEL_FAILURE + f'Channel split: item {k}: {what} is not on the GPU')
    if t.device != dev: raise RuntimeError(_KERNEL_FAILURE + f'Channel split: item {k}: {what} is on another device')


def split_plan_table(items) -> EqualizeTable:
    jobs = np.zeros(len(items), dtype=_SPLIT_PLAN_JOB)
    segs = np.zeros(sum(len(it[3]) for it in items), dtype=_EQ_SEGMENT)
    keep, records = [], []
    dev = items[0][0].device if items else None
    for k, (src_of, count, threshold, segments) in enumerate(items):
        if src_of.numel() % 2: raise RuntimeError(_KERNEL_FAILURE + f'Channel split: item {k}: SrcOf must hold 2 x C entries')
        _i32(src_of, 'SrcOf', k, dev, src_of.numel()); _i32(count, 'Count', k, dev, 1)
        keep += [src_of, count]
        jobs[k] = (segs.ctypes.data + len(records) * _EQ_SEGMENT.itemsize, src_of.data_ptr(), count.data_ptr(), len(segments), src_of.numel() // 2,
                   float(threshold), 0)
        for segment in segments:
            records.append(_segment_record(segment, k, dev))
            keep.append(segment[0])
    segs[:] = records
    return EqualizeTable(jobs, segs, keep, lib.ppqhip_split_plan_multi)


def split_apply_table(items) -> EqualizeTable:
    jobs = np.zeros(len(items), dtype=_SPLIT_APPLY_JOB)
    keep = []
    dev = items[0][0].device if items else None
    for k, (x, out, src_of, C, count, run) in enumerate(items):
        _eq_tensor(x, 'Value', k, dev); _eq_tensor(out, 'Out', k, dev)
        _i32(src_of, 'SrcOf', k, dev, src_of.numel())
        C, count, run = int(C), int(count), int(run)
        if C > 0 and run > 0 and x.numel() % (C * run) == 0 and C <= count <= 2 * C:
            if out.numel() != x.numel() // C * count or src_of.numel() < count:
                raise RuntimeError(_KERNEL_FAILURE + f'Channel split: item {k}: Out must hold {x.numel() // C * count} floats and SrcOf {count} entries')
        keep += [x, out, src_of]
        jobs[k] = (x.data_ptr(), out.data_ptr(), src_of.data_ptr(), x.numel(), run, C, count)
    return EqualizeTable(jobs, None, keep, lib.ppqhip_split_apply_multi)


def split_plan_launches(items) -> int:
    chunks = jobs = segs = 0
    for it in items:
        n = len(it[3])
        if jobs == 0 or jobs == SPLIT_MAX_JOBS or segs + n > SPLIT_MAX_SEGMENTS: chunks, jobs, segs = chunks + 1, 0, 0
        jobs, segs = jobs + 1, segs + n
    return 2 * chunks


def split_apply_launches(items) -> int:
    return (len(items) + SPLIT_MAX_JOBS - 1) // SPLIT_MAX_JOBS


def split_plan_multi(items) -> None:
    (items if isinstance(items, EqualizeTable) else split_plan_table(items)).run()


def split_apply_multi(items) -> None:
    (items if isinstance(items, EqualizeTable) else split_apply_table(items)).run()


_SSD_SCALES_JOB = np.dtype([('first', _EQ_SEGMENT), ('last', _EQ_SEGMENT), ('act_range', '<u8'), ('scales', '<u8'), ('ranges', '<u8'),
                            ('num_channel', '<i4'), ('channel_ratio', '<f4')])
_SSD_APPLY_JOB = np.dtype([('x', '<u8'), ('out', '<u8'), ('scales', '<u8'), ('n', '<i8'), ('run', '<i8'), ('inner', '<i8'),
                           ('group_out', '<i8'), ('num_channel', '<i8'), ('divide', '<i4'), ('reserved', '<i4')])
_FQ_MEASURE_JOB = np.dtype([('y', '<u8'), ('r', '<u8'), ('scale', '<u8'), ('offset', '<u8'), ('sums', '<u8'), ('rows', '<i8'),
                            ('count', '<i8'), ('num_channel', '<i8'), ('elem_per_channel', '<i8'), ('clip_min', '<i4'),
                            ('clip_max', '<i4'), ('rounding', '<i4'), ('reserved', '<i4')])


def ssd_scales_multi(items) -> None:
    if not items: return
    jobs = np.zeros(len(items), dtype=_SSD_SCALES_JOB)
    dev = items[0][2].device
    for k, (first, last, act, ratio, scales, ranges) in enumerate(items):
        C = act.numel()
        for what, t, n in (('ActRange', act, C), ('Scales', scales, 4 * C), ('Ranges', ranges, 2 * C)):
            _eq_tensor(t, what, k, dev)
            if t.numel() != n: raise RuntimeError(_KERNEL_FAILURE + f'SSD scales: item {k}: {what} must hold {n} floats')
        segs = [_segment_record(tuple(seg) + (1.0, False), k, dev, what) for what, seg in (('First', first), ('Last', last))]
        jobs[k] = (segs[0], segs[1], act.data_ptr(), scales.data_ptr(), ranges.data_ptr(), C, float(ratio))
    with _DeviceOf(items[0][2]):
        _raise(lib.ppqhip_ssd_scales_multi(jobs.ctypes.data, len(items), _stream()))


def ssd_apply_multi(items) -> None:
    if not items: return
    jobs = np.zeros(len(items), dtype=_SSD_APPLY_JOB)
    dev = items[0][0].device
    for k, (x, out, scales, run, inner, group_out, divide) in enumerate(items):
        _eq_tensor(x, 'Value', k, dev); _eq_tensor(out, 'Out', k, dev); _eq_tensor(scales, 'Scales', k, dev)
        if out.numel() != 4 * x.numel(): raise RuntimeError(_KERNEL_FAILURE + f'SSD apply: item {k}: Out must hold 4 x {x.numel()} floats')
        if scales.numel() % 4: raise RuntimeError(_KERNEL_FAILURE + f'SSD apply: item {k}: Scales must be [4, C]')
        jobs[k] = (x.data_ptr(), out.data_ptr(), scales.data_ptr(), x.numel(), int(run), int(inner), int(group_out),
                   scales.numel() // 4, 1 if divide else 0, 0)
    with _DeviceOf(items[0][0]):
        _raise(lib.ppqhip_ssd_apply_multi(jobs.ctypes.data, len(items), _stream()))


def fq_measure_rows_multi(items, sums=None) -> List[torch.Tensor]:
    if not items: return []
    dev = items[0][0].device
    if sums is None: sums = [torch.empty([it[0].shape[0], 4], dtype=torch.float64, device=dev) for it in items]
    jobs = np.zeros(len(items), dtype=_FQ_MEASURE_JOB)
    for k, ((y, r, scale, offset, axis, qmin, qmax, rounding), out) in enumerate(zip(items, sums)):
        rows, count = _rows_of(y, 'Value')
        if _rows_of(r, 'Real') != (rows, count): raise RuntimeError(_KERNEL_FAILURE + f'fq measure: item {k}: Value {tuple(y.shape)} and Real {tuple(r.shape)} do not match')
        _f32(scale, 'Scale'); _f32(offset, 'Offset')
        if axis is None: C, epc = 1, count
        else:
            if axis % y.dim() != 1: raise RuntimeError(_KERNEL_FAILURE + f'fq measure: item {k}: channel_axis must be 1, {axis} was given')
            C, epc = _geometry(y.shape, 1)
        if scale.numel() != C or offset.numel() != C or not scale.is_contiguous() or not offset.is_contiguous():
            raise RuntimeError(_KERNEL_FAILURE + f'fq measure: item {k}: Scale / Offset must be contiguous with {C} element(s)')
        if any(t.device != dev for t in (y, r, scale, offset, out)): raise RuntimeError(_KERNEL_FAILURE + f'fq measure: item {k} is on another device')
        if out.dtype != torch.float64 or out.numel() != rows * 4 or not out.is_contiguous():
            raise RuntimeError(_KERNEL_FAILURE + f'fq measure: item {k}: Sums must be a contiguous float64 [{rows}, 4]')
        jobs[k] = (y.data_ptr(), r.data_ptr(), scale.data_ptr(), offset.data_ptr(), out.data_ptr(), rows, count, C, epc,
                   int(qmin), int(qmax), int(rounding), 0)
    with _DeviceOf(items[0][0]):
        _raise(lib.ppqhip_fq_measure_rows_multi(jobs.ctypes.data, len(items), _stream()))
    return sums


_FETCH_JOB = np.dtype([('x', '<u8'), ('index', '<u8'), ('out', '<u8'), ('rows', '<i8'), ('row_len', '<i8'), ('count', '<i8')])
_MEASURE_JOB = np.dtype([('p', '<u8'), ('r', '<u8'), ('index', '<u8'), ('sums', '<u8'), ('rows', '<i8'), ('row_len', '<i8'),
                         ('count', '<i8')])
_FINISH_JOB = np.dtype([('sums', '<u8'), ('acc', '<u8'), ('row_out', '<u8'), ('rows', '<i8'), ('count', '<i8'),
                        ('method', '<i4'), ('reduce', '<i4')])
MEASURE_METHODS = {'snr': 0, 'mse': 1, 'cosine': 2}
MEASURE_REDUCES = {'mean': 0, 'max': 1}


def _rows_of(t: torch.Tensor, name: str):
    _f32(t, name)
    if not t.is_contiguous(): raise RuntimeError(_KERNEL_FAILURE + f'{name} is not contiguous')
    if t.dim() < 1: raise RuntimeError(_KERNEL_FAILURE + f'{name} has no batch dimension')
    return t.shape[0], t.numel() // t.shape[0]


def _index_of(index: torch.Tensor, row_len: int, dev) -> int:
    if index.dtype != torch.int32 or not index.is_cuda or not index.is_contiguous() or index.dim() != 1 or index.numel() == 0:
        raise RuntimeError(_KERNEL_FAILURE + 'Index must be a contiguous 1-D int32 tensor on the GPU')
# ... 1385 lines not shown
```

### ppq_amd/harness.py

```python
from typing import Callable, Dict, List, Optional

import torch
import torch.nn.functional as F

from .core import LinearQuantizationConfig, QuantizationStates, TensorQuantizationConfig, is_initial
from .core import QuantizationProperty as P
from .qfunction import PPQuantFunction

PASSIVE_OPERATIONS = {'MaxPool', 'GlobalMaxPool', 'Reshape', 'Flatten', 'Identity', 'Dropout', 'Slice', 'Pad', 'Resize',
                      'Split', 'Transpose', 'Interp', 'Squeeze', 'Unsqueeze'}
COMPUTING_OP = {'Conv', 'Gemm', 'ConvTranspose', 'MatMul'}


class Variable:
    def __init__(self, name: str, value: torch.Tensor = None, is_parameter: bool = False):
        self.name = name
        self.value = value
        self.stored_value = None
        self.is_parameter = is_parameter
        self.dest_ops: List['Operation'] = []
        self.source_op: Optional['Operation'] = None

    def __hash__(self): return hash(self.name)
    def __eq__(self, o): return isinstance(o, Variable) and o.name == self.name
# ... 75 lines not shown
        self.inputs: Dict[str, Variable] = {}
        self.outputs: Dict[str, Variable] = {}

    def create_variable(self, name: str, value=None, is_parameter=False) -> Variable:
        v = Variable(name, value, is_parameter)
        self.variables[name] = v
        return v

    def create_operation(self, op_type: str, name: str, inputs: List[Variable], attributes: dict = None) -> Variable:
        out = self.create_variable(name + '_out')
        op = Operation(name, op_type, attributes, list(inputs), [out])
        out.source_op = op
        for v in inputs: v.dest_ops.append(op)
        self.operations[name] = op
        return out

    def topological_sort(self) -> List[Operation]:
        return list(self.operations.values())


def _forward(op: Operation, x: List[torch.Tensor]):
    t, a = op.type, op.attributes
    if t == 'Conv':
        return F.conv2d(x[0], x[1], x[2] if len(x) > 2 else None, stride=a.get('strides', 1),
                        padding=a.get('pads', 0), groups=a.get('group', 1))
    if t == 'Gemm': return F.linear(x[0], x[1], x[2] if len(x) > 2 else None)
    if t == 'MatMul': return torch.matmul(x[0], x[1])
    if t == 'Relu': return F.relu(x[0])
    if t == 'Gelu': return F.gelu(x[0])
    if t == 'Add': return x[0] + x[1]
    if t == 'MaxPool': return F.max_pool2d(x[0], a['kernel_shape'], a.get('strides', 1), a.get('pads', 0))
    if t == 'GlobalAveragePool': return F.adaptive_avg_pool2d(x[0], 1)
    if t == 'Flatten': return torch.flatten(x[0], 1)
    if t == 'LayerNormalization': return F.layer_norm(x[0], x[0].shape[-1:], x[1], x[2])
    if t == 'Softmax': return F.softmax(x[0], dim=a.get('axis', -1))
    if t == 'Mul': return x[0] * (x[1] if len(x) > 1 else a['value'])
    if t == 'Reshape': return x[0].reshape(a['shape'])
    if t == 'Transpose': return x[0].permute(a['perm'])
    if t == 'Concat': return torch.cat([v.expand(x[-1].shape[0], *v.shape[1:]) if v.shape[0] == 1 else v for v in x],
                                       dim=a.get('axis', 1))
    if t == 'Slice': return x[0].narrow(a['axis'], a['start'], a['length'])
    if t == 'Resize': return F.interpolate(x[0], scale_factor=a.get('scale', 2), mode=a.get('mode', 'nearest'))
    raise NotImplementedError(f'Graph op: {op.name}({op.type}) has no backend implementation')


class EpilogueGroup:
    __slots__ = ('kind', 'ops', 'convs', 'add', 'relu')

    def __init__(self, kind, ops, convs, add, relu):
        self.kind, self.ops, self.convs, self.add, self.relu = kind, ops, convs, add, relu

    def __repr__(self): return f'{self.kind}({", ".join(op.name for op in self.ops)})'


def _in_cfg(op, i):
    return op.config.input_quantization_config[i] if isinstance(op, QuantableOperation) else None


def _out_cfg(op, i):
    return op.config.output_quantization_config[i] if isinstance(op, QuantableOperation) else None


def plan_epilogues(operations: List[Operation], hooks: Dict[str, object] = None, keep=(), passes_through: Callable = None,
                   grad_enabled: bool = False) -> List[EpilogueGroup]:
    if grad_enabled: return []
    from .observer import CalibrationHook
    hooks = hooks or {}
    keep = set(keep)
    if passes_through is None:
        def passes_through(c): return not QuantizationStates.is_activated(c.state)

    def through(*cfgs): return all(c is None or passes_through(c) for c in cfgs)

    def hooks_ok(members, unwritten):
        for op in members:
            h = hooks.get(op.name)
            if h is None: continue
            if type(h) is not CalibrationHook: return False
            if any(c is not None and c in h._observer_table for c in unwritten): return False
        return True

    def conv_ok(op):
        return (op.type == 'Conv' and len(op.inputs) == 3 and op.inputs[2].is_parameter and len(op.outputs) == 1
                and op.outputs[0].name not in keep)

    def only_feeds(v, op): return len(v.dest_ops) == 1 and v.dest_ops[0] is op

    def relu_after(op, i):
        if i >= len(operations): return None
        r = operations[i]
        out = op.outputs[0]
        if r.type != 'Relu' or len(r.inputs) != 1 or r.inputs[0] is not out or not only_feeds(out, r) or out.name in keep:
            return None
        return r

    def try_p2(i):
        for n_conv in (2, 1):
            j = i + n_conv
            if j + 1 >= len(operations): continue
            add, convs = operations[j], operations[i:j]
            if add.type != 'Add' or len(add.inputs) != 2 or len(add.outputs) != 1 or not all(conv_ok(c) for c in convs): continue
            by_out = {c.outputs[0].name: c for c in convs}
            x0, x1 = add.inputs
            if x0.name not in by_out or x0 is x1: continue
            if n_conv == 2 and x1.name not in by_out: continue
            ordered = [by_out[x0.name]] + ([by_out[x1.name]] if n_conv == 2 else [])
            if not all(only_feeds(c.outputs[0], add) for c in convs): continue
            relu = relu_after(add, j + 1)
            if relu is None: continue
            unwritten = (_out_cfg(add, 0), _in_cfg(relu, 0))
            between = [_out_cfg(c, 0) for c in convs] + [_in_cfg(add, 0), _in_cfg(add, 1)]
            if not through(*unwritten, *between): return None
            members = list(operations[i:j + 2])
            if not hooks_ok(members, unwritten): return None
            return EpilogueGroup('P2', members, ordered, add, relu)
        return None

    def try_p1(i):
        conv = operations[i]
        if not conv_ok(conv): return None
        relu = relu_after(conv, i + 1)
        if relu is None: return None
        unwritten = (_out_cfg(conv, 0), _in_cfg(relu, 0))
        if not through(*unwritten) or not hooks_ok([conv, relu], unwritten): return None
        return EpilogueGroup('P1', [conv, relu], [conv], None, relu)

    groups, i = [], 0
    while i < len(operations):
        g = try_p2(i) if operations[i].type == 'Conv' else None
        if g is None and operations[i].type == 'Conv': g = try_p1(i)
        if g is None:
            i += 1
            continue
        groups.append(g)
        i += len(g.ops)
    return groups


class TorchExecutor:
    def __init__(self, graph: BaseGraph, device: str = 'cuda'):
        self._graph = graph
        self._device = device
        self._default_quant_fn = PPQuantFunction
        self.cache_parameter_quantization = False
        self._param_cache: Dict[str, tuple] = {}
        self.fuse_parameter_quantization = True
        self._plans: list = []
        self._plan_signature = None
        self._plan_cache: Dict[tuple, list] = {}
        self._fused: Dict[tuple, torch.Tensor] = {}
        self._delegates: Dict[object, Callable] = {}
        self._overrides: Dict[str, Callable] = {}
        self.fuse_epilogues = True
        self._epilogue_cache: Dict[tuple, dict] = {}
        self.channels_last = False
        for v in graph.variables.values():
            if v.is_parameter and v.value is not None: v.value = v.value.to(device)

    def use_channels_last(self) -> 'TorchExecutor':
        self.channels_last = True
        for v in self._graph.variables.values():
            if v.is_parameter and isinstance(v.value, torch.Tensor) and v.value.dim() == 4:
                v.value = v.value.contiguous(memory_format=torch.channels_last)
        return self

    def _place(self, value: torch.Tensor) -> torch.Tensor:
        value = value.to(self._device)
        if self.channels_last and value.dim() == 4: value = value.contiguous(memory_format=torch.channels_last)
        return value

    def register_quantize_delegate(self, config, delegator: Callable) -> None:
        self._delegates[config] = delegator

    def remove_quantize_delegate(self, config) -> None:
        self._delegates.pop(config, None)

    def register_operation_override(self, op_name: str, fn: Callable) -> None:
        if op_name not in self._graph.operations: raise KeyError(f'register_operation_override: the graph has no operation {op_name!r}')
        if not callable(fn): raise TypeError(f'register_operation_override: fn must be callable, got {type(fn)}')
        self._overrides[op_name] = fn

    def remove_operation_override(self, op_name: str) -> None:
        self._overrides.pop(op_name, None)

    def quantize_function(self, tensor: torch.Tensor, config=None) -> torch.Tensor:
        if self._delegates and config in self._delegates:
            return self._delegates[config](tensor, config)
        return self._default_quant_fn(tensor, config)

    def forward_with_gradient(self, inputs, output_names: List[str] = None, hooks=None):
        return TorchExecutor.forward.__wrapped__(self, inputs, output_names, hooks)

    def partial_graph_forward(self, operations: List[Operation], feed_dict: Dict[str, torch.Tensor],
                              output_names: List[str], with_gradient: bool = False) -> List[torch.Tensor]:
        if not with_gradient:
            with torch.no_grad(): return self._partial_graph_forward(operations, feed_dict, output_names)
        return self._partial_graph_forward(operations, feed_dict, output_names)

    def _partial_graph_forward(self, operations, feed_dict, output_names):
        g = self._graph
        for name, value in feed_dict.items(): g.variables[name].value = self._place(value)
        results = [None] * len(output_names)
        self._fused_parameters(operations)
        plan, fused_done = self._epilogue_plan(operations, None, output_names), set()
        for op in operations:
            if op.name in fused_done: continue
            grp = plan.get(op.name)
            vals = self._run_epilogue(grp, lambda v: v.value, None) if grp is not None else None
            if vals is not None:
                for m in grp.ops:
                    fused_done.add(m.name)
                    for v in m.outputs:
                        v.value = vals[v.name]
                        if v.name in output_names: results[output_names.index(v.name)] = v.value
                continue
            raw_in = [v.value for v in op.inputs]
            if any(x is None for x in raw_in):
                raise ValueError(f'partial_graph_forward: input of {op.name} was not fed')
            override = self._overrides.get(op.name)
            if override is not None: outs = override(op, raw_in)
            else:
                if isinstance(op, QuantableOperation):
                    qin = [self._quantize_parameter(v, c) if v.is_parameter else self.quantize_function(x, c)
                           for v, x, c in zip(op.inputs, raw_in, op.config.input_quantization_config)]
                else: qin = raw_in
                outs = _forward(op, qin)
            outs = list(outs) if isinstance(outs, (list, tuple)) else [outs]
            if isinstance(op, QuantableOperation):
                outs = [self.quantize_function(y, c) for y, c in zip(outs, op.config.output_quantization_config)]
            for v, y in zip(op.outputs, outs):
                v.value = y
                if v.name in output_names: results[output_names.index(v.name)] = y
        for v in g.variables.values():
            if not v.is_parameter: v.value = None
        return results

    def _fused_parameters(self, operations=None) -> None:
        self._fused = {}
        if not self.fuse_parameter_quantization or self._default_quant_fn is not PPQuantFunction: return
        from .ffi import FloatingQuantizePlan, LinearQuantizePlan
        todo, sig = [], []
        for op in (self._graph.operations.values() if operations is None else operations):
            if not isinstance(op, QuantableOperation): continue
            for v, c in zip(op.inputs, op.config.input_quantization_config):
                if not (v.is_parameter and isinstance(v.value, torch.Tensor) and v.value.is_cuda): continue
                if not QuantizationStates.is_activated(c.state) or c in self._delegates: continue
                pol = c.policy
                floating = pol.has_property(P.FLOATING)
                if not (pol.has_property(P.LINEAR) or floating) or pol.has_property(P.DYNAMIC): continue
                if v.value.dtype != torch.float32 or v.value.requires_grad or v.value.numel() == 0: continue
                if not (isinstance(c.scale, torch.Tensor) and isinstance(c.offset, torch.Tensor)): continue
                axis = c.channel_axis if pol.has_property(P.PER_CHANNEL) else None
                if not LinearQuantizePlan.accepts(v.value, c.scale, c.offset, axis): continue
                rnd = int(getattr(c.rounding, 'value', c.rounding))
                todo.append((v, c, axis, rnd, floating))
                sig.append((v.name, id(c), v.value.data_ptr(), c.scale.data_ptr(), c.offset.data_ptr(), tuple(v.value.shape), c.scale.numel(),
                            axis, c.quant_min, c.quant_max, rnd, floating,
                            (c.exponent_bits, c.mantissa_bits) if floating else None))
        if not todo:
            self._plans, self._plan_signature = [], None
            return
        cached = self._plan_cache.get(tuple(sig))
        if cached is not None:
            self._plan_cache[tuple(sig)] = self._plan_cache.pop(tuple(sig))
            self._plans, self._plan_signature = cached, sig
        if sig != self._plan_signature:
            groups: Dict[tuple, list] = {}
            for item in todo: groups.setdefault((item[3], item[4]), []).append(item)
            self._plans = []
            for (rnd, floating), items in groups.items():
                if floating:
                    plan = FloatingQuantizePlan([(v.value, c.scale, c.offset, axis, c.exponent_bits, c.mantissa_bits,
                                                  c.quant_min, c.quant_max) for v, c, axis, _, _ in items], rounding=rnd)
                else:
                    plan = LinearQuantizePlan([(v.value, c.scale, c.offset, axis, c.quant_min, c.quant_max)
                                               for v, c, axis, _, _ in items], rounding=rnd)
                self._plans.append((plan, [(v.name, id(c)) for v, c, _, _, _ in items]))
            self._plan_signature = sig
            if len(self._plan_cache) >= 8: self._plan_cache.pop(next(iter(self._plan_cache)))
            self._plan_cache[tuple(sig)] = self._plans
        for plan, keys in self._plans:
            for key, out in zip(keys, plan.run()): self._fused[key] = out

    def _epilogue_plan(self, operations: List[Operation], hooks, output_names) -> Dict[str, EpilogueGroup]:
        if not self.fuse_epilogues or torch.is_grad_enabled() or self._default_quant_fn is not PPQuantFunction: return {}
        states = tuple(c.state for op in operations if isinstance(op, QuantableOperation)
                       for c in (*op.config.input_quantization_config, *op.config.output_quantization_config))
        sig = (tuple(op.name for op in operations), tuple((k, id(h)) for k, h in hooks.items()) if hooks else (),
               tuple(output_names or ()), tuple(id(c) for c in self._delegates), states, tuple(sorted(self._overrides)))
        plan = self._epilogue_cache.get(sig)
        if plan is None:
            delegates = self._delegates

            def passes_through(c): return not QuantizationStates.is_activated(c.state) and c not in delegates
            groups = plan_epilogues(operations, hooks, set(self._graph.outputs) | set(output_names or ()), passes_through)
            if self._overrides:
                groups = [g for g in groups if not any(m.name in self._overrides and not (hooks and m.name in hooks) for m in g.ops)]
            plan = {g.ops[0].name: g for g in groups}
            if len(self._epilogue_cache) >= 8: self._epilogue_cache.pop(next(iter(self._epilogue_cache)))
            self._epilogue_cache[sig] = plan
        return plan

    def _run_epilogue(self, grp: EpilogueGroup, raw_of: Callable, hooks) -> Optional[Dict[str, torch.Tensor]]:
        from .ffi import bias_act_, bias_add_act
        for conv in grp.convs:
            x, w = raw_of(conv.inputs[0]), conv.inputs[1].value
            if not (isinstance(x, torch.Tensor) and x.is_cuda and x.dtype == torch.float32 and x.dim() == 4
                    and isinstance(w, torch.Tensor) and w.dim() == 4): return None
            fmt = torch.channels_last if self.channels_last else torch.contiguous_format
            if not (x.is_contiguous(memory_format=fmt) and w.is_contiguous(memory_format=fmt)): return None
        if grp.add is not None:
            b_var = grp.add.inputs[1]
            if b_var.source_op not in grp.convs:
                b = raw_of(b_var)
                if not (isinstance(b, torch.Tensor) and b.is_cuda and b.dtype == torch.float32): return None
        hooks = hooks or {}
        ys, biases, qins = {}, {}, {}
        for conv in grp.ops[:len(grp.convs)]:
            raw_in = [raw_of(v) for v in conv.inputs]
            qin, in_cfgs = raw_in, None
            if isinstance(conv, QuantableOperation):
                in_cfgs = list(conv.config.input_quantization_config)
                qin = [self._quantize_parameter(v, c) if v.is_parameter else self.quantize_function(x, c)
                       for v, x, c in zip(conv.inputs, raw_in, in_cfgs)]
            hook = hooks.get(conv.name)
            if hook is not None: qin = hook.pre_forward_hook(inputs=raw_in, quant_inputs=qin, quant_configs=in_cfgs)
            a = conv.attributes
            ys[conv.name] = F.conv2d(qin[0], qin[1], None, stride=a.get('strides', 1), padding=a.get('pads', 0),
                                     groups=a.get('group', 1))
            biases[conv.name] = qin[2]
            qins[conv.name] = qin
        if grp.kind == 'P1':
            conv = grp.convs[0]
            y = ys[conv.name]
            if not bias_act_(y, biases[conv.name], relu=True):
                y.add_(biases[conv.name].view(1, -1, 1, 1)).relu_()
            tail = {conv.name: y, grp.relu.name: y}
        else:
            conv_a = grp.convs[0]
            a = ys[conv_a.name]
            conv_b = grp.convs[1] if len(grp.convs) > 1 else None
            b = ys[conv_b.name] if conv_b is not None else raw_of(grp.add.inputs[1])
            out = bias_add_act(a, biases[conv_a.name], b, biases[conv_b.name] if conv_b is not None else None, relu=True)
            if out is None:
                a.add_(biases[conv_a.name].view(1, -1, 1, 1))
                if conv_b is not None: b.add_(biases[conv_b.name].view(1, -1, 1, 1))
                out = F.relu(a + b)
            tail = {conv_a.name: a, grp.add.name: out, grp.relu.name: out}
            if conv_b is not None: tail[conv_b.name] = b
        values: Dict[str, torch.Tensor] = {}
        for op in grp.ops:
            hook = hooks.get(op.name)
            quantable = isinstance(op, QuantableOperation)
            if op.type != 'Conv':
                raw_in = [values[v.name] if v.name in values else raw_of(v) for v in op.inputs]
                qin, in_cfgs = raw_in, None
                if quantable:
                    in_cfgs = list(op.config.input_quantization_config)
                    qin = [self.quantize_function(x, c) for x, c in zip(raw_in, in_cfgs)]
                if hook is not None: hook.pre_forward_hook(inputs=raw_in, quant_inputs=qin, quant_configs=in_cfgs)
            outs = fp_outs = [tail[op.name]]
            out_cfgs = None
            if quantable:
                out_cfgs = list(op.config.output_quantization_config)
                outs = [self.quantize_function(y, c) for y, c in zip(outs, out_cfgs)]
            if hook is not None:
                outs = hook.post_forward_hook(outputs=fp_outs, quant_outputs=outs, quant_configs=out_cfgs)
            for v, y in zip(op.outputs, outs): values[v.name] = y
        return values

    def _quantize_parameter(self, var: Variable, config) -> torch.Tensor:
        hit = self._fused.get((var.name, id(config)))
        if hit is not None: return hit
        """A parameter and its scale do not change between calibration forwards, so its fake-quantised
        value is computed once and kept resident (the reference recomputes it every forward until
        ParameterBakingPass; same values, ppq/executor/torch.py:516-518).  The cache entry is keyed on
        the identity + version of value, scale and offset and on the config state."""
        if not self.cache_parameter_quantization or not QuantizationStates.is_activated(config.state):
            return self.quantize_function(var.value, config)
        key = (var.value.data_ptr(), var.value._version, id(config.scale), config.scale._version,
               id(config.offset), config.offset._version, int(getattr(config.state, 'value', config.state)))
        hit = self._param_cache.get(var.name)
        if hit is not None and hit[0] == key: return hit[1]
        q = self.quantize_function(var.value, config)
        self._param_cache[var.name] = (key, q)
        return q

    @ torch.no_grad()
    def forward_cached(self, inputs, output_names: List[str], cache: Dict[str, torch.Tensor]) -> List[torch.Tensor]:
        g = self._graph
        if isinstance(inputs, torch.Tensor): inputs = {next(iter(g.inputs)): inputs}
        elif isinstance(inputs, (list, tuple)): inputs = {k: v for k, v in zip(g.inputs, inputs)}
        for name, value in inputs.items():
            if name not in cache: cache[name] = self._place(value)
        need, stack = set(), [g.variables[n] for n in output_names]
        while stack:
            v = stack.pop()
            if v.name in cache or v.is_parameter: continue
            op = v.source_op
            if op is None: raise ValueError(f'forward_cached: graph input {v.name} was not fed')
            if op.name in need: continue
            need.add(op.name)
            stack.extend(op.inputs)
        ops = [op for op in g.topological_sort() if op.name in need]
        if ops: self._fused_parameters(ops)
        plan, fused_done = (self._epilogue_plan(ops, None, output_names) if ops else {}), set()
        for op in ops:
            if op.name in fused_done: continue
            grp = plan.get(op.name)
            vals = (self._run_epilogue(grp, lambda v: v.value if v.is_parameter else cache[v.name], None)
                    if grp is not None else None)
            if vals is not None:
                hidden = grp.relu.inputs[0].name
                for m in grp.ops:
                    fused_done.add(m.name)
                    for v in m.outputs:
                        if v.name != hidden: cache[v.name] = vals[v.name]
                continue
            raw_in = [v.value if v.is_parameter else cache[v.name] for v in op.inputs]
            override = self._overrides.get(op.name)
            if override is not None: outs = override(op, raw_in)
            else:
                if isinstance(op, QuantableOperation):
                    qin = [self._quantize_parameter(v, c) if v.is_parameter else self.quantize_function(x, c)
                           for v, x, c in zip(op.inputs, raw_in, op.config.input_quantization_config)]
                else: qin = raw_in
                outs = _forward(op, qin)
            outs = list(outs) if isinstance(outs, (list, tuple)) else [outs]
            if isinstance(op, QuantableOperation):
                outs = [self.quantize_function(y, c) for y, c in zip(outs, op.config.output_quantization_config)]
            for v, y in zip(op.outputs, outs): cache[v.name] = y
        return [cache[n] for n in output_names]

    @ torch.no_grad()
    def forward(self, inputs, output_names: List[str] = None, hooks: Dict[str, object] = None) -> List[torch.Tensor]:
        g = self._graph
        if isinstance(inputs, torch.Tensor): inputs = {next(iter(g.inputs)): inputs}
        elif isinstance(inputs, (list, tuple)): inputs = {k: v for k, v in zip(g.inputs, inputs)}
        for name, value in inputs.items(): g.variables[name].value = self._place(value)
        stop_early = output_names is not None and not hooks
        if output_names is None: output_names = list(g.outputs)
        results = [None] * len(output_names)
        visited = set()
        self._fused_parameters()
        ops = g.topological_sort()
        plan, fused_done = self._epilogue_plan(ops, hooks, output_names), set()

        def finish(op, outs):
            for v, y in zip(op.outputs, outs):
                v.value = y
                if v.name in output_names: results[output_names.index(v.name)] = y
            visited.add(op.name)
            for v in op.inputs:
                if not v.is_parameter and all(d.name in visited for d in v.dest_ops): v.value = None

        for op in ops:
            if op.name in fused_done: continue
            grp = plan.get(op.name)
            vals = self._run_epilogue(grp, lambda v: v.value, hooks) if grp is not None else None
            if vals is not None:
                for m in grp.ops:
                    fused_done.add(m.name)
                    finish(m, [vals[v.name] for v in m.outputs])
                if stop_early and all(r is not None for r in results): break
                continue
            hook = hooks.get(op.name) if hooks else None
            raw_in = [v.value for v in op.inputs]
            qin = raw_in
            quantable = isinstance(op, QuantableOperation)
            override = self._overrides.get(op.name) if hook is None else None
            if override is not None: outs = override(op, raw_in)
            else:
                if quantable:
                    in_cfgs = list(op.config.input_quantization_config)
                    qin = [self._quantize_parameter(v, c) if v.is_parameter else self.quantize_function(x, c)
                           for v, x, c in zip(op.inputs, raw_in, in_cfgs)]
                if hook is not None:
                    qin = hook.pre_forward_hook(inputs=raw_in, quant_inputs=qin, quant_configs=in_cfgs)
                outs = _forward(op, qin)
            outs = list(outs) if isinstance(outs, (list, tuple)) else [outs]
            fp_outs = outs
            if quantable:
                out_cfgs = list(op.config.output_quantization_config)
                outs = [self.quantize_function(y, c) for y, c in zip(outs, out_cfgs)]
            if hook is not None:
                outs = hook.post_forward_hook(outputs=fp_outs, quant_outputs=outs, quant_configs=out_cfgs)
            finish(op, outs)
            if stop_early and all(r is not None for r in results): break
        for v in g.variables.values():
            if not v.is_parameter: v.value = None
        return results


def quantize_graph(graph: BaseGraph, activation_algorithm: str = 'kl', per_channel_weight: bool = True,
                   symmetrical: bool = True, weight_symmetrical: bool = True, num_of_bits: int = 8,
                   hist_bins: int = None, fp8: bool = False, passive_bias: bool = False) -> None:
    qmin, qmax = (-(2 ** (num_of_bits - 1)), 2 ** (num_of_bits - 1) - 1) if symmetrical else (0, 2 ** num_of_bits - 1)
    wmin, wmax = (-(2 ** (num_of_bits - 1)), 2 ** (num_of_bits - 1) - 1) if weight_symmetrical else (0, 2 ** num_of_bits - 1)

    def act_cfg():
        if fp8:
            from .core import FloatingQuantizationConfig
            return FloatingQuantizationConfig(calibration='floating')
        c = LinearQuantizationConfig(symmetrical=symmetrical, quant_min=qmin, quant_max=qmax, num_of_bits=num_of_bits,
                                     calibration=activation_algorithm)
        if hist_bins is not None: c.detail['OBSERVER_KL_HIST_BINS_MANUL_OVERRIDE'] = hist_bins
        return c

    for name, op in list(graph.operations.items()):
        in_cfgs = []
        for i, v in enumerate(op.inputs):
            if v.is_parameter and op.type in COMPUTING_OP and i == 1:
                in_cfgs.append(LinearQuantizationConfig(symmetrical=weight_symmetrical, quant_min=wmin, quant_max=wmax,
                                                        num_of_bits=num_of_bits, calibration='minmax',
                                                        channel_axis=0 if per_channel_weight else None))
            elif v.is_parameter and passive_bias and not fp8 and op.type in COMPUTING_OP and i == 2:
                in_cfgs.append(LinearQuantizationConfig(symmetrical=True, quant_min=-(2 ** 31 - 1), quant_max=2 ** 31 - 1, num_of_bits=32,
                                                        calibration=None, channel_axis=0 if per_channel_weight else None))
                in_cfgs[-1].state = QuantizationStates.PASSIVE_INIT
            elif v.is_parameter:
                c = act_cfg(); c.state = QuantizationStates.FP32
                in_cfgs.append(c)
            else:
                in_cfgs.append(act_cfg())
        qop = QuantableOperation(op, OperationQuantizationConfig(in_cfgs, [act_cfg() for _ in op.outputs]))
        for v in qop.inputs: v.dest_ops[v.dest_ops.index(op)] = qop
        for v in qop.outputs: v.source_op = qop
        graph.operations[name] = qop
    ops = list(graph.operations.values())
    for op in ops:
        for v, c in zip(op.inputs, op.config.input_quantization_config):
            if v.source_op is not None and is_initial(c):
                src = v.source_op
                c.dominated_by = src.config.output_quantization_config[src.outputs.index(v)]
    for op in ops:
        out = op.outputs[0]
        if op.type in COMPUTING_OP | {'Add'} and len(out.dest_ops) == 1 and out.dest_ops[0].type in {'Relu', 'Gelu'}:
            op.config.output_quantization_config[0].dominated_by = out.dest_ops[0].config.output_quantization_config[0]
        if op.type in PASSIVE_OPERATIONS:
            first = op.config.input_quantization_config[0]
            if first.dominated_by is not op.config.output_quantization_config[0].dominated_by:
                op.config.output_quantization_config[0].dominated_by = first
            else: op.config.output_quantization_config[0].state = QuantizationStates.OVERLAPPED


from .parameters import ParameterBakingPass, ParameterQuantizePass


def _he(shape, gen) -> torch.Tensor:
    fan_in = shape[1] * (shape[2] * shape[3] if len(shape) == 4 else 1)
    return torch.randn(shape, generator=gen) * (2.0 / fan_in) ** 0.5


def resnet50_graph(seed: int = 0, num_classes: int = 1000) -> BaseGraph:
    gen = torch.Generator().manual_seed(seed)
    g = BaseGraph('resnet50')
    x = g.create_variable('input')
    g.inputs['input'] = x
    n = [0]

    def conv(inp, cin, cout, k, stride=1, pad=0, relu=True, tag='conv'):
        n[0] += 1
        w = g.create_variable(f'{tag}{n[0]}_w', _he([cout, cin, k, k], gen), True)
        b = g.create_variable(f'{tag}{n[0]}_b', torch.randn(cout, generator=gen) * 0.05, True)
        y = g.create_operation('Conv', f'{tag}{n[0]}', [inp, w, b], {'strides': stride, 'pads': pad})
        if relu: y = g.create_operation('Relu', f'relu{n[0]}', [y])
        return y

    y = conv(x, 3, 64, 7, 2, 3)
    y = g.create_operation('MaxPool', 'maxpool', [y], {'kernel_shape': 3, 'strides': 2, 'pads': 1})
    cin = 64
    for stage, (blocks, width) in enumerate(zip([3, 4, 6, 3], [64, 128, 256, 512])):
        for blk in range(blocks):
            stride = 2 if (blk == 0 and stage > 0) else 1
            identity = y
            z = conv(y, cin, width, 1)
            z = conv(z, width, width, 3, stride, 1)
            z = conv(z, width, width * 4, 1, relu=False)
            if blk == 0:
                identity = conv(y, cin, width * 4, 1, stride, 0, relu=False, tag='down')
            n[0] += 1
            z = g.create_operation('Add', f'add{n[0]}', [z, identity])
            y = g.create_operation('Relu', f'relu{n[0]}', [z])
            cin = width * 4
    y = g.create_operation('GlobalAveragePool', 'gap', [y])
    y = g.create_operation('Flatten', 'flatten', [y])
    w = g.create_variable('fc_w', torch.randn([num_classes, 2048], generator=gen) * (1.0 / 2048) ** 0.5, True)
    b = g.create_variable('fc_b', torch.zeros(num_classes), True)
    y = g.create_operation('Gemm', 'fc', [y, w, b])
    g.outputs[y.name] = y
    return g


def yolov6s_graph(seed: int = 0, num_classes: int = 80) -> BaseGraph:
    gen = torch.Generator().manual_seed(seed)
    g = BaseGraph('yolov6s')
    x = g.create_variable('input')
    g.inputs['input'] = x
    n = [0]

    def conv(inp, cin, cout, k=3, stride=1, relu=True, tag='conv'):
        n[0] += 1
        a = (6.0 / (cin * k * k)) ** 0.5
        w = g.create_variable(f'{tag}{n[0]}_w', (torch.rand([cout, cin, k, k], generator=gen) * 2 - 1) * a, True)
        b = g.create_variable(f'{tag}{n[0]}_b', torch.randn(cout, generator=gen) * 0.05, True)
        y = g.create_operation('Conv', f'{tag}{n[0]}', [inp, w, b], {'strides': stride, 'pads': k // 2})
        if relu: y = g.create_operation('Relu', f'relu{n[0]}', [y])
        return y

    def rep(inp, c, repeats):
        for _ in range(repeats): inp = conv(inp, c, c, 3, tag='rep')
        return inp

    def cat(name, vs): return g.create_operation('Concat', name, vs, {'axis': 1})

    y = conv(x, 3, 32, 3, 2, tag='stem')
    feats, cin = [], 32
    for stage, (c, r) in enumerate(zip([64, 128, 256, 512], [2, 4, 6, 2])):
        y = conv(y, cin, c, 3, 2, tag=f's{stage}_down')
        y = rep(y, c, r)
        cin = c
        feats.append(y)
    p = conv(feats[3], 512, 256, 1, tag='sppf_in')
    m1 = g.create_operation('MaxPool', 'sppf_pool1', [p], {'kernel_shape': 5, 'strides': 1, 'pads': 2})
    m2 = g.create_operation('MaxPool', 'sppf_pool2', [m1], {'kernel_shape': 5, 'strides': 1, 'pads': 2})
    m3 = g.create_operation('MaxPool', 'sppf_pool3', [m2], {'kernel_shape': 5, 'strides': 1, 'pads': 2})
    c5 = conv(cat('sppf_cat', [p, m1, m2, m3]), 1024, 512, 1, tag='sppf_out')
    c3, c4 = feats[1], feats[2]
    r5 = conv(c5, 512, 128, 1, tag='reduce5')
    u5 = g.create_operation('Resize', 'up5', [r5], {'scale': 2})
    p4 = rep(conv(cat('cat_p4', [u5, c4]), 128 + 256, 128, 3, tag='p4_in'), 128, 3)
    r4 = conv(p4, 128, 64, 1, tag='reduce4')
    u4 = g.create_operation('Resize', 'up4', [r4], {'scale': 2})
    p3 = rep(conv(cat('cat_p3', [u4, c3]), 64 + 128, 64, 3, tag='p3_in'), 64, 3)
    d3 = conv(p3, 64, 64, 3, 2, tag='down3')
    n4 = rep(conv(cat('cat_n4', [d3, r4]), 64 + 64, 128, 3, tag='n4_in'), 128, 3)
    d4 = conv(n4, 128, 128, 3, 2, tag='down4')
    n5 = rep(conv(cat('cat_n5', [d4, r5]), 128 + 128, 256, 3, tag='n5_in'), 256, 3)
    for name, f, c in (('s8', p3, 64), ('s16', n4, 128), ('s32', n5, 256)):
        stem = conv(f, c, c, 1, tag=f'head_{name}_stem')
        cls = conv(conv(stem, c, c, 3, tag=f'head_{name}_cls'), c, num_classes, 1, relu=False, tag=f'head_{name}_cls_out')
        box = conv(conv(stem, c, c, 3, tag=f'head_{name}_box'), c, 4, 1, relu=False, tag=f'head_{name}_box_out')
        g.outputs[cls.name] = cls
        g.outputs[box.name] = box
    _unit_variance_init(g, torch.rand(2, 3, 96, 96, generator=gen))
    return g


@ torch.no_grad()
def _unit_variance_init(g: BaseGraph, sample: torch.Tensor) -> None:
    values = {next(iter(g.inputs)): sample}
    for op in g.operations.values():
        xs = [v.value if v.is_parameter else values[v.name] for v in op.inputs]
        y = _forward(op, xs)
        if op.type == 'Conv':
            std = float(y.std())
            if std > 0:
                op.inputs[1].value = op.inputs[1].value / std
                if len(op.inputs) > 2: op.inputs[2].value = op.inputs[2].value / std
                y = y / std
        values[op.outputs[0].name] = y


def small_cnn_graph(seed: int = 0, width: int = 16) -> BaseGraph:
    gen = torch.Generator().manual_seed(seed)
    g = BaseGraph('small_cnn')
    x = g.create_variable('input'); g.inputs['input'] = x

    def conv(inp, cin, cout, name, relu):
        w = g.create_variable(name + '_w', _he([cout, cin, 3, 3], gen), True)
        b = g.create_variable(name + '_b', torch.randn(cout, generator=gen) * 0.1, True)
        y = g.create_operation('Conv', name, [inp, w, b], {'strides': 1, 'pads': 1})
# ... 107 lines not shown
```

### ppq_amd/observer.py

```python
from typing import Dict, List, Optional, Sequence, Tuple

import weakref

import numpy as np
import torch

from .core import (OBSERVER_FLOATING_MSE_FETCHES, OBSERVER_ISOTONE_OBSERVER_AXIS, OBSERVER_KL_HIST_BINS, OBSERVER_KL_HIST_BINS_MANUL_OVERRIDE,
                   OBSERVER_MIN_SCALE, OBSERVER_MIN_SCALE_MANUL_OVERRIDE, OBSERVER_MSE_HIST_BINS,
                   OBSERVER_PERCENTILE, OBSERVER_PERCENTILE_MANUL_OVERRIDE, is_initial, set_activated)
from .core import QuantizationProperty as P
from .core import RoundingPolicy
from .ffi import CUDA, quantile_hint
from .round import ppq_numerical_round, ppq_round_to_power_of_2


def minmax_to_scale_offset(min_val: float, max_val: float, config,
                           scale_threshold: float = OBSERVER_MIN_SCALE) -> Tuple[float, float]:
    if OBSERVER_MIN_SCALE_MANUL_OVERRIDE in config.detail:
        scale_threshold = config.detail[OBSERVER_MIN_SCALE_MANUL_OVERRIDE]
    scale, offset = 1, 0
    if min_val > 0: min_val = 0
    if max_val < 0: max_val = 0
    if config.policy.has_property(P.ASYMMETRICAL):
        range = float(max_val - min_val)
        scale = range / (config.quant_max - config.quant_min)
        scale = max(scale, scale_threshold)
        offset = ppq_numerical_round(float(-min_val / scale))
    elif config.policy.has_property(P.SYMMETRICAL):
        range = 2 * float(max(abs(max_val), abs(min_val)))
        scale = range / (config.quant_max - config.quant_min)
        scale = max(scale, scale_threshold)
        offset = 0
    else:
        raise TypeError('Tensor Min Max Observer Excepts either ASYMMETRICAL or SYMMETRICAL quantization config.')
    if config.policy.has_property(P.POWER_OF_2):
        scale = ppq_round_to_power_of_2(scale, policy=RoundingPolicy.ROUND_UP)
    return scale, offset


def minmax_to_scale_offset_channels(mins: np.ndarray, maxs: np.ndarray, config,
                                    scale_threshold: float = OBSERVER_MIN_SCALE) -> Tuple[list, list]:
    if config.policy.has_property(P.POWER_OF_2) or mins.dtype != np.float32 or maxs.dtype != np.float32:
        pairs = [minmax_to_scale_offset(a, b, config, scale_threshold) for a, b in zip(mins, maxs)]
        return [p[0] for p in pairs], [p[1] for p in pairs]
    if OBSERVER_MIN_SCALE_MANUL_OVERRIDE in config.detail:
        scale_threshold = config.detail[OBSERVER_MIN_SCALE_MANUL_OVERRIDE]
    zero = np.float32(0)
    lo = np.where(mins > 0, zero, mins)
    hi = np.where(maxs < 0, zero, maxs)
    levels = config.quant_max - config.quant_min
    if config.policy.has_property(P.ASYMMETRICAL):
        with np.errstate(over='ignore', divide='ignore', invalid='ignore'):
            scale = (hi - lo).astype(np.float64) / levels
            scale = np.where(scale_threshold > scale, scale_threshold, scale)
            offset = np.rint(((-lo) / scale.astype(np.float32)).astype(np.float64))
        return scale.tolist(), [int(v) for v in offset.tolist()]
    if config.policy.has_property(P.SYMMETRICAL):
        a, b = np.abs(hi), np.abs(lo)
        m = np.where(b > a, b, a)
        scale = 2 * m.astype(np.float64) / levels
        scale = np.where(scale_threshold > scale, scale_threshold, scale)
        return scale.tolist(), [0] * int(scale.size)
    raise TypeError('Tensor Min Max Observer Excepts either ASYMMETRICAL or SYMMETRICAL quantization config.')


_DEFERRED_SETS: Optional[list] = None


def _set_per_tensor(config, scale: float, offset: float, device) -> None:
    if _DEFERRED_SETS is not None:
        _DEFERRED_SETS.append((config, scale, offset, device))
        return
    config.scale = torch.tensor([scale], dtype=torch.float32, device=device).squeeze(0)
    config.offset = torch.tensor([offset], dtype=torch.float32, device=device).squeeze(0)
    set_activated(config)


def _flush_deferred_sets(pending: list) -> None:
    by_dev: Dict[object, list] = {}
    for item in pending: by_dev.setdefault(torch.device(item[3]), []).append(item)
    for dev, items in by_dev.items():
        chunks = [np.asarray(v, dtype=np.float32).reshape(-1) for _, s, o, _ in items for v in (s, o)]
        flat = torch.from_numpy(np.concatenate(chunks)).to(dev)
        pos = 0
        for k, (config, s, _, _) in enumerate(items):
            if isinstance(s, (list, tuple)):
                C = len(s)
                config.scale, config.offset = flat[pos: pos + C], flat[pos + C: pos + 2 * C]
                pos += 2 * C
            else:
                config.scale, config.offset = flat[pos], flat[pos + 1]
                pos += 2
            set_activated(config)


class ObservationQueue:
    def __init__(self, max_pending_bytes: int = 4 << 30):
        self._minmax = []
        self._minmax_c = []
        self._hist = {}
        self._quantile = {}
        self._bytes = 0
        self._max = max_pending_bytes
        self.launches = 0
        self.recorder: Optional[list] = None

    def __len__(self):
        return (len(self._minmax) + len(self._minmax_c) + sum(len(v) for v in self._hist.values())
                + sum(len(v) for v in self._quantile.values()))

    def _grow(self, value) -> None:
        self._bytes += value.numel() * 4
        if self._bytes > self._max: self.flush()

    def add_minmax(self, value: torch.Tensor, slots: torch.Tensor) -> None:
        self._minmax.append((value, slots))
        self._grow(value)

    def add_minmax_c(self, value: torch.Tensor, channel_axis: int, mins: torch.Tensor, maxs: torch.Tensor, fresh: bool) -> None:
        if any(m.data_ptr() == mins.data_ptr() for _, _, m, _, _ in self._minmax_c): self.flush()
        self._minmax_c.append((value, channel_axis, mins, maxs, bool(fresh)))
        self._grow(value)

    def add_hist(self, value: torch.Tensor, rows: torch.Tensor, asymmetric: bool, p0: float, p1: float = 0.0) -> None:
        self._hist.setdefault((bool(asymmetric), rows.shape[1], value.device), []).append((value, rows, p0, p1))
        self._grow(value)

    def add_quantile(self, value: torch.Tensor, q: float, hint: Optional[torch.Tensor] = None) -> torch.Tensor:
        dest = torch.empty(2, dtype=torch.float32, device=value.device)
        self._quantile.setdefault((float(q), value.device), []).append((value, dest, hint))
        self._grow(value)
        return dest

    def flush(self) -> None:
        if self._quantile:
            pending, self._quantile = self._quantile, {}
            for (q, _), items in pending.items():
                hints, seen = [h for _, _, h in items], set()
                for k in range(len(hints) - 1, -1, -1):
                    if hints[k] is None: continue
                    key = hints[k].data_ptr()
                    if key in seen: hints[k] = None
                    else: seen.add(key)
                CUDA.Quantile_Multi([v for v, _, _ in items], q, [d for _, d, _ in items], hints)
                self.launches += 1
        if self._minmax:
            by_dev = {}
            for v, sl in self._minmax: by_dev.setdefault(v.device, []).append((v, sl))
            self._minmax = []
            for items in by_dev.values():
                CUDA.MinMax_T_Slots_Multi([v for v, _ in items], [sl for _, sl in items])
                self.launches += 1
        if self._minmax_c:
            by_dev = {}
            for it in self._minmax_c: by_dev.setdefault(it[0].device, []).append(it)
            self._minmax_c = []
            for dev, items in by_dev.items():
                CUDA.MinMax_C_Multi([i[0] for i in items], [i[1] for i in items], [i[2] for i in items],
                                    [i[3] for i in items], [i[4] for i in items])
                self.launches += 1
        if self._hist:
            pending, self._hist = self._hist, {}
            for (asym, _, _), items in pending.items():
                vs, rows = [i[0] for i in items], [i[1] for i in items]
                if asym:
                    CUDA.Histogram_Asymmetric_T_Rows_Multi([i[2] for i in items], [i[3] for i in items], vs, rows)
                else:
                    CUDA.Histogram_T_Rows_Multi(vs, rows, [i[2] for i in items])
                self.launches += 1
        self._bytes = 0


SIBLING_PREFETCH = False
_LIVE_OBSERVERS: "weakref.WeakSet" = weakref.WeakSet()
_PREFETCHING = False


def _prefetch_siblings(ob) -> None:
    global _PREFETCHING
    if not SIBLING_PREFETCH or _PREFETCHING: return
    _PREFETCHING = True
    try:
        def device_of(o):
            t = getattr(o, '_hist', None) if getattr(o, '_hist', None) is not None else getattr(o, '_range', None)
            return None if t is None else t.device
        dev = device_of(ob)
        sibs = [o for o in list(_LIVE_OBSERVERS) if isinstance(o, TorchMinMaxObserver) and is_initial(o._quant_cfg) and device_of(o) == dev]
        if ob not in sibs: sibs.append(ob)
        _prefetch(sibs)
    finally:
        _PREFETCHING = False


class BaseTensorObserver:
    queue: Optional[ObservationQueue] = None

    def __init__(self, watch_on, quant_cfg):
        self._watch_on = watch_on
        self._quant_cfg = quant_cfg
        _LIVE_OBSERVERS.add(self)

    def _drain(self) -> None:
        if self.queue is not None and len(self.queue): self.queue.flush()

    def observe(self, value):
        raise NotImplementedError('Implement this function first.')

    def render_quantization_config(self):
        raise NotImplementedError('Implement this function first.')

    def __str__(self) -> str:
        return ('PPQ Tensor Observer (' + self.__class__.__name__ + ') mount on variable ' +
                getattr(self._watch_on, 'name', str(self._watch_on)) + ' observing algorithm: ' +
                str(self._quant_cfg.observer_algorithm))

    def report(self) -> str:
        return ''

    def pending_range(self) -> Optional[torch.Tensor]:
        return None

    def take_range(self, host: np.ndarray) -> None:
        """Receive the host copy of ``pending_range()`` (fetched for all observers at once)."""

    def reducible(self) -> List[Tuple[torch.Tensor, str]]:
        return []

    def gatherable(self) -> List[torch.Tensor]:
        return []

    def take_gathered(self, merged: List[torch.Tensor]) -> None:
        pass


_RANGE_SEEDS: Dict[object, tuple] = {}


def _range_seed(device) -> tuple:
    hit = _RANGE_SEEDS.get(device)
    if hit is None:
        one = torch.tensor([float('inf'), float('-inf')], dtype=torch.float32, device=device)
        hit = _RANGE_SEEDS[device] = (one, one.repeat(CUDA.minmax_slots(), 1).contiguous())
    return hit


class TorchMinMaxObserver(BaseTensorObserver):
    def __init__(self, watch_on, quant_cfg):
        super().__init__(watch_on, quant_cfg)
        self._range: Optional[torch.Tensor] = None
        self._slots: Optional[torch.Tensor] = None
        self._slots_dirty = False
        self._queued_c = False
        self._host_range: Optional[np.ndarray] = None
        self._observed = False

    @ torch.no_grad()
    def observe(self, value: torch.Tensor):
        assert isinstance(value, torch.Tensor), 'TorchMinMaxObserver can only deal with torch Tensor values'
        assert value.numel() > 0, (f'You are observing an empty tensor({getattr(self._watch_on, "name", "")}).')
        if not is_initial(self._quant_cfg): return
        cfg = self._quant_cfg
        if cfg.policy.has_property(P.PER_TENSOR):
            if self._range is None:
                seed = _range_seed(value.device)
                self._range = seed[0].clone()
                self._slots = seed[1].clone()
            if self.queue is not None and value.is_cuda: self.queue.add_minmax(value, self._slots)
            else: CUDA.MinMax_T_Slots(value, self._slots)
            self._slots_dirty = True
        elif cfg.policy.has_property(P.PER_CHANNEL):
            queued = (self.queue is not None and value.is_cuda and CUDA.minmax_c_outer_is_one(value, cfg.channel_axis))
            fresh = False
            if self._range is None:
                C = value.shape[cfg.channel_axis]
                self._range = torch.empty((2, C), dtype=torch.float32, device=value.device)
                fresh = queued and CUDA.minmax_c_fresh_ok(value, cfg.channel_axis)
                if not fresh: self._range[0].fill_(float('inf')); self._range[1].fill_(float('-inf'))
            if queued:
                self.queue.add_minmax_c(value, cfg.channel_axis, self._range[0], self._range[1], fresh)
                self._queued_c = True
            else: CUDA.MinMax_C(value, cfg.channel_axis, self._range[0], self._range[1])
        else:
            raise TypeError('Min-max Observer only work with per-tensor or per-channel quantize policy.')
        self._observed = True
        self._host_range = None

    def _fold(self) -> None:
        if self._queued_c:
            self._drain()
            self._queued_c = False
        if self._slots_dirty:
            self._drain()
            CUDA.MinMax_Slots_Finish(self._slots, self._range)
            self._slots_dirty = False

    def pending_range(self):
        if not (is_initial(self._quant_cfg) and self._observed): return None
        self._fold()
        return self._range

    def take_range(self, host: np.ndarray) -> None:
        self._host_range = host

    def reducible(self):
        if self._range is None: return []
        self._fold()
        if self._range.ndim == 1: return [(self._range[0:1], 'min'), (self._range[1:2], 'max')]
        return [(self._range[0], 'min'), (self._range[1], 'max')]

    def _range_on_host(self) -> np.ndarray:
        if not self._observed:
            raise ValueError('Can not render quantization config yet, Observer data collator is empty. '
                             'Invoke observe() function before render config.')
        if self._host_range is None: _prefetch_siblings(self)
        if self._host_range is None:
            self._fold()
            self._host_range = self._range.cpu().numpy()
        return self._host_range

    def render_quantization_config(self):
        if not is_initial(self._quant_cfg): return
        cfg = self._quant_cfg
        r = self._range_on_host()
        device = self._range.device
        if cfg.policy.has_property(P.PER_TENSOR):
            scale, offset = minmax_to_scale_offset(min_val=float(r[0]), max_val=float(r[1]), config=cfg)
            _set_per_tensor(cfg, scale, offset, device)
        elif cfg.policy.has_property(P.PER_CHANNEL):
            scales, offsets = minmax_to_scale_offset_channels(np.ascontiguousarray(r[0]), np.ascontiguousarray(r[1]), cfg)
            if _DEFERRED_SETS is not None:
                _DEFERRED_SETS.append((cfg, scales, offsets, device))
                return
            cfg.scale = torch.tensor(scales, dtype=torch.float32, device=device)
            cfg.offset = torch.tensor(offsets, dtype=torch.float32, device=device)
            set_activated(cfg)
        else:
            raise TypeError('Min-max Observer only work with per-tensor or per-channel quantize policy.')


class TorchHistObserver(TorchMinMaxObserver):
    def __init__(self, watch_on, quant_cfg, hist_bins: int = OBSERVER_KL_HIST_BINS):
        self._phase = 'Detecting Minmax'
        self._hist = None
        self._rows = None
        self._rows_dirty = False
        self._hist_scale = None
        self._min = None
        self._max = None
        self._losses: Optional[np.ndarray] = None
        if OBSERVER_KL_HIST_BINS_MANUL_OVERRIDE in quant_cfg.detail:
            hist_bins = quant_cfg.detail[OBSERVER_KL_HIST_BINS_MANUL_OVERRIDE]
        self._hist_bins = hist_bins
        super().__init__(watch_on, quant_cfg)

    def observe(self, value: torch.Tensor):
        if not is_initial(self._quant_cfg): return
        assert value.numel() > 0, (f'You are observing an empty tensor({getattr(self._watch_on, "name", "")}).')
        if self._phase == 'Detecting Minmax':
            if self.queue is not None and self.queue.recorder is not None and value.is_cuda:
                self.queue.recorder.append((self, value))
            return super().observe(value)
        elif self._phase == 'Collating Hist':
            self._losses = None
            if getattr(self, '_best', None) is not None: self._best = None
            if self._hist is None:
                self._hist = torch.zeros(size=(self._hist_bins,), dtype=torch.int32, device=value.device)
                if self._hist_bins <= 16384:
                    self._rows = torch.zeros(size=(CUDA.hist_rows(), self._hist_bins), dtype=torch.int32,
                                             device=value.device)
            if self._quant_cfg.policy.has_property(P.ASYMMETRICAL):
                if self._rows is not None:
                    if self.queue is not None: self.queue.add_hist(value, self._rows, True, self._min, self._max)
                    else: CUDA.Histogram_Asymmetric_T_Rows(self._min, self._max, tensor=value, rows=self._rows)
                    self._rows_dirty = True
                else:
                    CUDA.Histogram_Asymmetric_T(self._min, self._max, tensor=value, histogram=self._hist)
            elif self._quant_cfg.policy.has_property(P.SYMMETRICAL):
                if self._rows is not None:
                    if self.queue is not None: self.queue.add_hist(value, self._rows, False, self._hist_scale)
                    else: CUDA.Histogram_T_Rows(tensor=value, rows=self._rows, scale=self._hist_scale)
                    self._rows_dirty = True
                else:
                    CUDA.Histogram_T(tensor=value, histogram=self._hist, scale=self._hist_scale)
            else:
                raise TypeError('Quantization Property is invalid, expect either ASYMMETRICAL or SYMMETRICAL config here.')

    def pending_range(self):
        return super().pending_range() if self._phase == 'Detecting Minmax' else None

    def _fold_hist(self) -> None:
        if self._rows_dirty:
            self._drain()
            CUDA.Histogram_Rows_Finish(self._rows, self._hist)
            self._rows_dirty = False
            if self._rows.is_cuda: self._rows.record_stream(torch.cuda.current_stream(self._rows.device))
            self._rows = None

    def histogram(self) -> Optional[torch.Tensor]:
        self._fold_hist()
        return self._hist

    def reducible(self):
        if self._phase == 'Detecting Minmax': return super().reducible()
        return [(self.histogram(), 'sum')] if self._hist is not None else []

    search_kind = 'kl'

    def search_key(self):
        return ('kl', self._hist_bins, self._quant_cfg.num_of_bits)

    def take_losses(self, losses: np.ndarray) -> None:
        self._losses = losses

    def hist_to_scale_offset(self, histogram: torch.Tensor, hist_bins: int, hist_scale: float, config,
                             scale_threshold: float = OBSERVER_MIN_SCALE) -> Tuple[float, int]:
        if config.policy.has_property(P.ASYMMETRICAL):
            raise PermissionError('KL observer is not designed for ASYMMETRICAL quantization')
        if OBSERVER_MIN_SCALE_MANUL_OVERRIDE in config.detail:
            scale_threshold = config.detail[OBSERVER_MIN_SCALE_MANUL_OVERRIDE]
        quant_bins = 2 ** (config.num_of_bits - 1)
        if self._losses is None: _prefetch_siblings(self)
        if self._losses is None:
            self._losses = CUDA.KLLosses(histogram, config.num_of_bits).cpu().numpy()[0]
        losses = [{'kl': float(kl), 'bin_range': (j + 1) * quant_bins} for j, kl in enumerate(self._losses)]
        best_bin_range = sorted(losses, key=lambda x: x['kl'])[0]['bin_range']
        scale, offset = (best_bin_range / self._hist_bins) * hist_scale * (self._hist_bins / quant_bins), 0
        scale = max(scale, scale_threshold)
        if config.policy.has_property(P.POWER_OF_2):
            scale = ppq_round_to_power_of_2(scale, policy=RoundingPolicy.ROUND_HALF_UP)
        return scale, offset

    def render_quantization_config(self):
        if not is_initial(self._quant_cfg): return
        if not self._quant_cfg.policy.has_property(P.PER_TENSOR):
            raise ValueError('Hist observer can only apply with per-tensor quantization config.')
        if self._phase == 'Detecting Minmax':
            r = self._range_on_host()
            min_val, max_val = float(r[0]), float(r[1])
            if self._quant_cfg.policy.has_property(P.SYMMETRICAL):
                hist_range = float(max(abs(max_val), abs(min_val)))
            else:
                hist_range = max_val - min_val
            self._min = min_val
            self._max = max_val
            self._hist_scale = hist_range / self._hist_bins
            self._phase = 'Collating Hist'
        elif self._phase == 'Collating Hist':
            if self._hist is None:
                raise ValueError('Can not render quantization config yet, histogram is empty. '
                                 'Invoke observe() function before render config.')
            scale, offset = self.hist_to_scale_offset(histogram=self.histogram(), hist_bins=self._hist_bins,
                                                      hist_scale=self._hist_scale, config=self._quant_cfg)
            _set_per_tensor(self._quant_cfg, scale, offset, self._hist.device)


class ChannelwiseKLObserver(TorchHistObserver):
    def __init__(self, watch_on, quant_cfg, hist_bins: int = OBSERVER_KL_HIST_BINS):
        super().__init__(watch_on, quant_cfg, hist_bins)
        if not quant_cfg.policy.has_property(P.PER_CHANNEL) or not quant_cfg.policy.has_property(P.SYMMETRICAL):
            raise TypeError('ChannelwiseKLObserver needs a symmetrical per-channel config.')
        self._scales_dev: Optional[torch.Tensor] = None

    def observe(self, value: torch.Tensor):
        if not is_initial(self._quant_cfg): return
        assert value.numel() > 0, (f'You are observing an empty tensor({getattr(self._watch_on, "name", "")}).')
        if self._phase == 'Detecting Minmax':
            return TorchMinMaxObserver.observe(self, value)
        C = value.shape[self._quant_cfg.channel_axis]
        if self._hist is None:
            self._hist = torch.zeros(size=(C, self._hist_bins), dtype=torch.int32, device=value.device)
        CUDA.Histogram_C_Scales(value, self._quant_cfg.channel_axis, self._hist, self._scales_dev)

    def histogram(self): return self._hist

    def render_quantization_config(self):
        cfg = self._quant_cfg
        if not is_initial(cfg): return
        if self._phase == 'Detecting Minmax':
            r = self._range_on_host()
            hs = [float(max(abs(float(hi)), abs(float(lo)))) / self._hist_bins for lo, hi in zip(r[0], r[1])]
            self._hist_scale = hs
            self._scales_dev = torch.tensor(hs, dtype=torch.float32, device=self._range.device)
            self._phase = 'Collating Hist'
            return
        if self._hist is None:
            raise ValueError('Can not render quantization config yet, histogram is empty. '
                             'Invoke observe() function before render config.')
        losses = CUDA.KLLosses(self._hist, cfg.num_of_bits).cpu().numpy()
        scales = []
        for c in range(self._hist.shape[0]):
            self._losses = losses[c]
            scale, _ = self.hist_to_scale_offset(self._hist[c], self._hist_bins, self._hist_scale[c], cfg)
            scales.append(scale)
        self._losses = None
        cfg.scale = torch.tensor(scales, dtype=torch.float32, device=self._hist.device)
        cfg.offset = torch.zeros(len(scales), dtype=torch.float32, device=self._hist.device)
        set_activated(cfg)


class TorchPercentileObserver(BaseTensorObserver):
    def __init__(self, watch_on, quant_cfg):
        super().__init__(watch_on, quant_cfg)
        if OBSERVER_PERCENTILE_MANUL_OVERRIDE not in quant_cfg.detail:
            self._percentile = OBSERVER_PERCENTILE
        else: self._percentile = quant_cfg.detail[OBSERVER_PERCENTILE_MANUL_OVERRIDE]
        self._percentile_collector = []
        self._sum: Optional[torch.Tensor] = None
        self._hint: Optional[torch.Tensor] = None

    @ torch.no_grad()
    def observe(self, value: torch.Tensor):
        if not is_initial(self._quant_cfg): return
        assert value is not None, ('You are observing an Empty Tensor. '
                                   '(This Error is usually due to you have a wrong Quantizer configuration.)')
        assert value.numel() > 0, (f'You are observing an empty tensor({getattr(self._watch_on, "name", "")}).')
        assert isinstance(value, torch.Tensor), 'TorchMinMaxObserver can only deal with torch Tensor values'
        if self._quant_cfg.policy.has_property(P.PER_TENSOR):
            if value.is_cuda and (self._hint is None or self._hint.device != value.device):
                self._hint = quantile_hint(value.device)
            if self.queue is not None and value.is_cuda:
                self._percentile_collector.append(self.queue.add_quantile(value, self._percentile, self._hint).view(1, -1))
            else:
                self._percentile_collector.append(CUDA.Quantile_Hinted(value, self._percentile, self._hint).view(1, -1))
        elif self._quant_cfg.policy.has_property(P.PER_CHANNEL):
            raise PermissionError('Percentile observer can not deal with per channel quantization.')
        else:
            raise TypeError('Min-max Observer only work with per-tensor or per-channel quantize policy.')

    def _fold(self):
        self._drain()
        if self._percentile_collector:
            stacked = torch.cat(self._percentile_collector, dim=0).float()
            part = torch.cat([stacked.sum(dim=0), stacked.new_tensor([float(stacked.shape[0])])])
            self._sum = part if self._sum is None else self._sum + part
            self._percentile_collector = []

    def reducible(self):
        self._fold()
        return [(self._sum, 'sum')] if self._sum is not None else []

    def render_quantization_config(self):
        if not is_initial(self._quant_cfg): return
        if self._quant_cfg.policy.has_property(P.PER_TENSOR):
            single_shard = self._sum is None
            if single_shard and len(self._percentile_collector) == 0:
                raise ValueError('Can not render quantization config yet, Observer data collator is empty. '
                                 'Invoke observe() function before render config.')
            self._drain()
            if single_shard:
                device = self._percentile_collector[-1].device
                mean = torch.cat(self._percentile_collector, dim=0).float().mean(dim=0).cpu()
            else:
                self._fold()
                device = self._sum.device
                mean = (self._sum[:2] / self._sum[2]).cpu()
            scale, offset = minmax_to_scale_offset(min_val=mean[1].item(), max_val=mean[0].item(),
                                                   config=self._quant_cfg)
            _set_per_tensor(self._quant_cfg, scale, offset, device)
        elif self._quant_cfg.policy.has_property(P.PER_CHANNEL):
            raise PermissionError('Percentile observer can not deal with per channel quantization.')
        else:
            raise TypeError('Min-max Observer only work with per-tensor or per-channel quantize policy.')


class TorchMSEObserver(TorchHistObserver):
    search_kind = 'mse'

    def __init__(self, watch_on, quant_cfg, bins: int = OBSERVER_MSE_HIST_BINS):
        super().__init__(watch_on, quant_cfg)
        self._hist_bins = bins
        self._best: Optional[np.ndarray] = None

    def search_key(self):
        cfg = self._quant_cfg
        return ('mse', self._hist_bins, cfg.quant_min, cfg.quant_max, cfg.policy.has_property(P.SYMMETRICAL))

    def take_best(self, best: np.ndarray) -> None:
        self._best = best

    def compute_mse_loss(self, histogram: list, start: int, step: int, end: int) -> float:
        return CUDA.compute_mse_loss(histogram=histogram, start=start, step=step, end=end)

    def hist_to_scale_offset(self, histogram: torch.Tensor, hist_bins: int, hist_scale: float, config,
                             scale_threshold: float = OBSERVER_MIN_SCALE) -> Tuple[float, int]:
        if OBSERVER_MIN_SCALE_MANUL_OVERRIDE in config.detail:
            scale_threshold = config.detail[OBSERVER_MIN_SCALE_MANUL_OVERRIDE]
        if config.policy.has_property(P.PER_CHANNEL):
            raise PermissionError('Torch Mse observer do not support PER_CHANNEL policy now, please wait.')
        symmetrical = config.policy.has_property(P.SYMMETRICAL)
        if self._best is None: _prefetch_siblings(self)
        if self._best is None:
            dev = histogram.device
            self._best = CUDA.MseSearch(histogram.reshape(1, -1),
                                        torch.tensor([hist_scale], dtype=torch.float64, device=dev),
                                        torch.tensor([self._min], dtype=torch.float64, device=dev),
                                        config.quant_min, config.quant_max, symmetrical).cpu().numpy()[0]
        best_start, best_end = int(self._best[0]), int(self._best[1])
        if not symmetrical:
            range_min, range_max = (best_start * hist_scale) + self._min, (best_end * hist_scale) + self._min
        else:
            range_min, range_max = -(best_end * hist_scale), (best_end * hist_scale)
        return minmax_to_scale_offset(range_min, range_max, config, scale_threshold)


class ChannelwiseMSEObserver(TorchMSEObserver):
    def __init__(self, watch_on, quant_cfg, bins: int = OBSERVER_MSE_HIST_BINS):
        super().__init__(watch_on, quant_cfg, bins)
        if not quant_cfg.policy.has_property(P.PER_CHANNEL):
            raise TypeError('ChannelwiseMSEObserver needs a per-channel config.')
        self._mins_dev = self._maxs_dev = self._scales_dev = None

    def observe(self, value: torch.Tensor):
        if not is_initial(self._quant_cfg): return
        assert value.numel() > 0, (f'You are observing an empty tensor({getattr(self._watch_on, "name", "")}).')
        if self._phase == 'Detecting Minmax':
            return TorchMinMaxObserver.observe(self, value)
        cfg = self._quant_cfg
        C = value.shape[cfg.channel_axis]
        if self._hist is None:
            self._hist = torch.zeros(size=(C, self._hist_bins), dtype=torch.int32, device=value.device)
        if cfg.policy.has_property(P.ASYMMETRICAL):
            CUDA.Histogram_Asymmetric_C_Ranges(value, cfg.channel_axis, self._hist, self._mins_dev, self._maxs_dev)
        else:
            CUDA.Histogram_C_Scales(value, cfg.channel_axis, self._hist, self._scales_dev)

    def histogram(self): return self._hist

    def reducible(self):
        if self._phase == 'Detecting Minmax': return TorchMinMaxObserver.reducible(self)
        return [(self._hist, 'sum')] if self._hist is not None else []

    def render_quantization_config(self):
        cfg = self._quant_cfg
        if not is_initial(cfg): return
        sym = cfg.policy.has_property(P.SYMMETRICAL)
        if self._phase == 'Detecting Minmax':
            r = self._range_on_host()
            self._min = [float(v) for v in r[0]]
            self._max = [float(v) for v in r[1]]
            self._hist_scale = [(float(max(abs(hi), abs(lo))) if sym else (hi - lo)) / self._hist_bins
                                for lo, hi in zip(self._min, self._max)]
            dev = self._range.device
            self._mins_dev = torch.tensor(self._min, dtype=torch.float32, device=dev)
            self._maxs_dev = torch.tensor(self._max, dtype=torch.float32, device=dev)
            self._scales_dev = torch.tensor(self._hist_scale, dtype=torch.float32, device=dev)
            self._phase = 'Collating Hist'
            return
        if self._hist is None:
            raise ValueError('Can not render quantization config yet, histogram is empty. '
                             'Invoke observe() function before render config.')
        dev = self._hist.device
        best = CUDA.MseSearch(self._hist, torch.tensor(self._hist_scale, dtype=torch.float64, device=dev),
                              torch.tensor(self._min, dtype=torch.float64, device=dev), cfg.quant_min, cfg.quant_max,
                              sym).cpu().numpy()
        scale_threshold = cfg.detail.get(OBSERVER_MIN_SCALE_MANUL_OVERRIDE, OBSERVER_MIN_SCALE)
        scales, offsets = [], []
        for c in range(self._hist.shape[0]):
            start, end, hs = int(best[c][0]), int(best[c][1]), self._hist_scale[c]
            if sym: range_min, range_max = -(end * hs), (end * hs)
            else: range_min, range_max = (start * hs) + self._min[c], (end * hs) + self._min[c]
            s_, o_ = minmax_to_scale_offset(range_min, range_max, cfg, scale_threshold)
            scales.append(s_); offsets.append(o_)
        cfg.scale = torch.tensor(scales, dtype=torch.float32, device=dev)
        cfg.offset = torch.tensor(offsets, dtype=torch.float32, device=dev)
        set_activated(cfg)


class ConstantObserver(BaseTensorObserver):
    def __init__(self, watch_on, quant_cfg):
        super().__init__(watch_on, quant_cfg)
        self._value_shape = None
        self._value_device = None

    @ torch.no_grad()
    def observe(self, value: torch.Tensor):
        if not is_initial(self._quant_cfg): return
        self._value_shape = value.shape
        self._value_device = value.device

    def render_quantization_config(self):
        if not is_initial(self._quant_cfg): return
        device = self._value_device
        cfg = self._quant_cfg
        if cfg.policy.has_property(P.FLOATING):
            if cfg.policy.has_property(P.PER_TENSOR):
                _set_per_tensor(cfg, 1.0, 0.0, device)
            elif cfg.policy.has_property(P.PER_CHANNEL):
                num = self._value_shape[cfg.channel_axis]
# ... 354 lines not shown
```

Before: 3535 samples/s.

## Fuse per-tensor min/max observation into conv bias/residual/ReLU epilogue kernels

Adds epilogue kernels that apply bias, residual add and ReLU while also folding per-tensor min/max into per-block observer slots. The observer queue records these tensors as prepaid so the later hook does not re-read them. This removes a separate full read pass over each activation during the min/max phase of KL calibration. The cost is extra kernel variants, prepay bookkeeping tied to data pointers, and persistent-grid kernels that may run differently from the old elementwise epilogue.

New measurement: 3615 samples/s, median of 6. +2.2%, better.

```diff
diff --git a/include/ppq_hip.h b/include/ppq_hip.h
--- a/include/ppq_hip.h
+++ b/include/ppq_hip.h
@@ -225,6 +225,13 @@
                     int relu, void* stream);
 int ppqhip_bias_add_act(float* a, const float* bias_a, float* b, const float* bias_b, float* out,
                         int64_t n, int64_t num_channel, int64_t elem_per_channel, int relu, void* stream);
+
+#define PPQHIP_NOT_FUSED 1
+int ppqhip_bias_act_stats(float* y, const float* bias, int64_t n, int64_t num_channel, int64_t elem_per_channel,
+                          int relu, float* slots_y, void* stream);
+int ppqhip_bias_add_act_stats(float* a, const float* bias_a, float* b, const float* bias_b, float* out,
+                              int64_t n, int64_t num_channel, int64_t elem_per_channel, int relu,
+                              float* slots_a, float* slots_b, float* slots_out, void* stream);
 
 typedef struct ppqhip_adaround_job {
     const float* w;
diff --git a/ppq_amd/_lib.py b/ppq_amd/_lib.py
--- a/ppq_amd/_lib.py
+++ b/ppq_amd/_lib.py
@@ -13,6 +13,9 @@
 c_vp = ctypes.c_void_p
 
 ABI_VERSION = 4
+
+
+NOT_FUSED = 1
 
 
 class ProfEntry(ctypes.Structure):
@@ -38,6 +41,9 @@
     'ppqhip_lsq_finish_multi': (c_int, [c_vp, c_int, c_vp]),
     'ppqhip_bias_act': (c_int, [c_f32p, c_f32p, c_i64, c_i64, c_i64, c_int, c_vp]),
     'ppqhip_bias_add_act': (c_int, [c_f32p, c_f32p, c_f32p, c_f32p, c_f32p, c_i64, c_i64, c_i64, c_int, c_vp]),
+    'ppqhip_bias_act_stats': (c_int, [c_f32p, c_f32p, c_i64, c_i64, c_i64, c_int, c_f32p, c_vp]),
+    'ppqhip_bias_add_act_stats': (c_int, [c_f32p, c_f32p, c_f32p, c_f32p, c_f32p, c_i64, c_i64, c_i64, c_int, c_f32p, c_f32p,
+                                          c_f32p, c_vp]),
     'ppqhip_fq_float_t': (c_int, [c_f32p, c_f32p, c_f32p, c_f32p, c_i64, c_int, c_int, c_flt, c_flt, c_int, c_vp]),
     'ppqhip_fq_float_c': (c_int, [c_f32p, c_f32p, c_f32p, c_f32p, c_i64, c_i64, c_i64, c_int, c_int, c_flt, c_flt,
                                   c_int, c_vp]),
diff --git a/ppq_amd/csrc/epilogue.hip b/ppq_amd/csrc/epilogue.hip
--- a/ppq_amd/csrc/epilogue.hip
+++ b/ppq_amd/csrc/epilogue.hip
@@ -1,4 +1,5 @@
 #include "common.hpp"
+#include "minmax_fold.hpp"
 
 namespace ppqhip {
 namespace {
@@ -49,15 +50,33 @@
                        bias[channel_of(i + 3, epc, nc)]);
 }
 
+template <typename T>
+struct EpStored { T a, b, out; };
+
 template <bool RESID, bool BIAS_B, bool RELU>
-__device__ __forceinline__ void epilogue_elem(const EpArgs& p, uint32_t i, const FastDiv& epc) {
+__device__ __forceinline__ EpStored<float> epilogue_elem(const EpArgs& p, uint32_t i, const FastDiv& epc) {
+    EpStored<float> s{};
     const uint32_t c = channel_of(i, epc, p.nc);
     const float x = p.a[i] + p.bias_a[c];
-    if (!RESID) { p.a[i] = act(x, RELU); return; }
-    p.a[i] = x;
+    if (!RESID) { p.a[i] = s.a = act(x, RELU); return s; }
+    p.a[i] = s.a = x;
     float y = p.b[i];
-    if (BIAS_B) { y = y + p.bias_b[c]; p.b[i] = y; }
-    p.out[i] = act(x + y, RELU);
+    if (BIAS_B) { y = y + p.bias_b[c]; p.b[i] = s.b = y; }
+    p.out[i] = s.out = act(x + y, RELU);
+    return s;
+}
+
+template <bool RESID, bool BIAS_B, bool RELU>
+__device__ __forceinline__ EpStored<float4> epilogue_vec(float4* a4, float4* b4, float4* o4, uint32_t vv, const float4& a,
+                                                         const float4& ba, const float4& b, const float4& bb) {
+    EpStored<float4> s{};
+    const float4 x = add4(a, ba);
+    if (!RESID) { a4[vv] = s.a = act4<RELU>(x); return s; }
+    a4[vv] = s.a = x;
+    float4 y = b;
+    if (BIAS_B) { y = add4(y, bb); b4[vv] = s.b = y; }
+    o4[vv] = s.out = act4<RELU>(add4(x, y));
+    return s;
 }
 
 template <int U, bool RESID, bool BIAS_B, bool RELU, bool PLANE>
@@ -66,7 +85,7 @@
     float4* a4 = reinterpret_cast<float4*>(p.a);
     float4* b4 = reinterpret_cast<float4*>(p.b);
     float4* o4 = reinterpret_cast<float4*>(p.out);
-    float4 a[U], ba[U], b[U], bb[U];
+    float4 a[U], ba[U], b[U]{}, bb[U]{};
 #pragma unroll
     for (int k = 0; k < U; k++) {
         const uint32_t vv = min(base + k * kBlock, p.nvec - 1);
@@ -79,12 +98,7 @@
     for (int k = 0; k < U; k++) {
         const uint32_t vv = base + k * kBlock;
         if (vv >= p.nvec) continue;
-        const float4 x = add4(a[k], ba[k]);
-        if (!RESID) { a4[vv] = act4<RELU>(x); continue; }
-        a4[vv] = x;
-        float4 y = b[k];
-        if (BIAS_B) { y = add4(y, bb[k]); b4[vv] = y; }
-        o4[vv] = act4<RELU>(add4(x, y));
+        epilogue_vec<RESID, BIAS_B, RELU>(a4, b4, o4, vv, a[k], ba[k], b[k], bb[k]);
     }
     if (!PLANE && blockIdx.x == 0 && (int)threadIdx.x < p.ntail)
         epilogue_elem<RESID, BIAS_B, RELU>(p, p.tail + threadIdx.x, p.epc);
@@ -122,6 +136,101 @@
 #undef PPQ_LAUNCH_EP
 }
 
+struct EpSinks { float* slots[3]; };
+constexpr int kEpStatBlock = 512;
+constexpr int kEpStatWgPerCu = 2;
+
+template <int U, bool RESID, bool BIAS_B, bool RELU, bool PLANE>
+__global__ __launch_bounds__(kEpStatBlock, (kEpStatBlock * kEpStatWgPerCu + 255) / 256)
+void epilogue_stats_kernel(EpArgs p, EpSinks sk) {
+    __shared__ float lds[32];
+    constexpr int NS = RESID ? 3 : 1;
+    constexpr uint32_t kTile = (uint32_t)kEpStatBlock * U;
+    const uint32_t G = gridDim.x, g = blockIdx.x;
+    const uint32_t full = p.nvec / kTile, tiles = full + (p.nvec > full * kTile ? 1u : 0u);
+    uint32_t t, t_end;
+    even_split(tiles, G, g, t, t_end);
+    float4* a4 = reinterpret_cast<float4*>(p.a);
+    float4* b4 = reinterpret_cast<float4*>(p.b);
+    float4* o4 = reinterpret_cast<float4*>(p.out);
+
+    bool live[NS];
+    float mn[NS], mx[NS];
+#pragma unroll
+    for (int k = 0; k < NS; k++) {
+        live[k] = sk.slots[k] != nullptr && (k != 1 || BIAS_B);
+        mn[k] = INFINITY; mx[k] = -INFINITY;
+    }
+    auto feed4 = [&](const EpStored<float4>& s) {
+        if (live[0]) minmax_fold4(mn[0], mx[0], s.a);
+        if (RESID) {
+            if (BIAS_B && live[1]) minmax_fold4(mn[1], mx[1], s.b);
+            if (live[NS - 1]) minmax_fold4(mn[NS - 1], mx[NS - 1], s.out);
+        }
+    };
+    auto feed1 = [&](const EpStored<float>& s) {
+        if (live[0]) minmax_fold1(mn[0], mx[0], s.a);
+        if (RESID) {
+            if (BIAS_B && live[1]) minmax_fold1(mn[1], mx[1], s.b);
+            if (live[NS - 1]) minmax_fold1(mn[NS - 1], mx[NS - 1], s.out);
+        }
+    };
+
+    struct Tile { float4 a[U], ba[U], b[U], bb[U]; };
+    auto fetch = [&](Tile& T, uint32_t tile) {
+        const uint32_t base = tile * kTile + threadIdx.x;
+#pragma unroll
+        for (int u = 0; u < U; u++) {
+            const uint32_t vv = base + u * kEpStatBlock;
+            T.a[u] = a4[vv];
+            T.ba[u] = bias4<PLANE>(p.bias_a, vv, p.epc, p.nc);
+            if (RESID) T.b[u] = b4[vv];
+            if (BIAS_B) T.bb[u] = bias4<PLANE>(p.bias_b, vv, p.epc, p.nc);
+        }
+    };
+    auto consume = [&](const Tile& T, uint32_t tile) {
+        const uint32_t base = tile * kTile + threadIdx.x;
+#pragma unroll
+        for (int u = 0; u < U; u++)
+            feed4(epilogue_vec<RESID, BIAS_B, RELU>(a4, b4, o4, base + u * kEpStatBlock, T.a[u], T.ba[u], T.b[u], T.bb[u]));
+    };
+    const uint32_t tf = min(t_end, full);
+    if (t < tf) {
+        Tile ta{}, tb{};
+        fetch(ta, t);
+        for (;;) {
+            fetch(tb, min(t + 1, tf - 1));
+            consume(ta, t);
+            if (++t >= tf) break;
+            fetch(ta, min(t + 1, tf - 1));
+            consume(tb, t);
+            if (++t >= tf) break;
+        }
+    }
+    if (t < t_end) {
+        const uint32_t base = t * kTile + threadIdx.x;
+#pragma unroll
+        for (int u = 0; u < U; u++) {
+            const uint32_t vv = base + u * kEpStatBlock;
+            const uint32_t vc = min(vv, p.nvec - 1);
+            const float4 a = a4[vc], ba = bias4<PLANE>(p.bias_a, vc, p.epc, p.nc);
+            float4 b{}, bb{};
+            if (RESID) b = b4[vc];
+            if (BIAS_B) bb = bias4<PLANE>(p.bias_b, vc, p.epc, p.nc);
+            if (vv < p.nvec) feed4(epilogue_vec<RESID, BIAS_B, RELU>(a4, b4, o4, vv, a, ba, b, bb));
+        }
+    }
+    if (!PLANE && g == G - 1 && (int)threadIdx.x < p.ntail)
+        feed1(epilogue_elem<RESID, BIAS_B, RELU>(p, p.tail + threadIdx.x, p.epc));
+#pragma unroll
+    for (int k = 0; k < NS; k++) {
+        if (!live[k]) continue;
+        minmax_block_fold(mn[k], mx[k], lds);
+        if (threadIdx.x == 0) minmax_slot_fold(sk.slots[k] + 2 * g, mn[k], mx[k]);
+        __syncthreads();
+    }
+}
+
 int validate(int64_t n, int64_t C, int64_t epc, const char* what) {
     if (n <= 0 || n > 0x7fffffffLL) {
         set_error("%s: n=%lld is empty or has more than 2^31 - 1 elements", what, (long long)n);
@@ -133,6 +242,36 @@
         return PPQHIP_ERR_INVALID_VALUE;
     }
     return PPQHIP_OK;
+}
+
+template <bool RESID, bool BIAS_B>
+int launch_epilogue_stats(EpArgs p, int64_t n, int64_t C, int64_t epc, int relu, bool aligned, EpSinks sk, const char* what,
+                          hipStream_t st) {
+    if ((!sk.slots[0] && !sk.slots[1] && !sk.slots[2]) || !aligned || n < 4) return PPQHIP_NOT_FUSED;
+    p.nc = make_fastdiv((uint32_t)C);
+    p.nvec = (uint32_t)(n >> 2);
+    p.tail = p.nvec * 4u;
+    p.ntail = (int)(n & 3);
+    const bool plane = (epc % 4 == 0);
+    p.epc = make_fastdiv((uint32_t)(plane ? epc / 4 : epc));
+    const bool small = n <= kEpSmallElems;
+    const uint32_t tile = (uint32_t)kEpStatBlock * (small ? kEpSmallU : kEpTileU), tiles = (p.nvec + tile - 1) / tile;
+    const uint32_t cap = (uint32_t)(num_cu() * kEpStatWgPerCu);
+    const uint32_t grid = tiles < cap ? tiles : cap;
+#define PPQ_LAUNCH_EPS(U, RELU, PLANE)                                                                                    \
+    hipLaunchKernelGGL((epilogue_stats_kernel<U, RESID, BIAS_B, RELU, PLANE>), dim3(grid), dim3(kEpStatBlock), 0, st, p, sk)
+    switch ((small ? 0 : 4) | (relu ? 2 : 0) | (plane ? 1 : 0)) {
+        case 0: PPQ_LAUNCH_EPS(kEpSmallU, false, false); break;
+        case 1: PPQ_LAUNCH_EPS(kEpSmallU, false, true); break;
+        case 2: PPQ_LAUNCH_EPS(kEpSmallU, true, false); break;
+        case 3: PPQ_LAUNCH_EPS(kEpSmallU, true, true); break;
+        case 4: PPQ_LAUNCH_EPS(kEpTileU, false, false); break;
+        case 5: PPQ_LAUNCH_EPS(kEpTileU, false, true); break;
+        case 6: PPQ_LAUNCH_EPS(kEpTileU, true, false); break;
+        default: PPQ_LAUNCH_EPS(kEpTileU, true, true); break;
+    }
+#undef PPQ_LAUNCH_EPS
+    return finish_launch(what);
 }
 
 }
@@ -173,4 +312,29 @@
     return finish_launch("bias_add_act");
 }
 
-}
+int ppqhip_bias_act_stats(float* y, const float* bias, int64_t n, int64_t num_channel, int64_t elem_per_channel, int relu,
+                          float* slots_y, void* stream) {
+    if (int st = validate(n, num_channel, elem_per_channel, "bias_act_stats")) return st;
+    if (!y || !bias) { set_error("bias_act_stats: null pointer"); return PPQHIP_ERR_INVALID_VALUE; }
+    EpArgs p{};
+    p.a = y; p.bias_a = bias;
+    return launch_epilogue_stats<false, false>(p, n, num_channel, elem_per_channel, relu, aligned16(y), EpSinks{{slots_y, nullptr, nullptr}},
+                                               "bias_act_stats", (hipStream_t)stream);
+}
+
+int ppqhip_bias_add_act_stats(float* a, const float* bias_a, float* b, const float* bias_b, float* out, int64_t n,
+                              int64_t num_channel, int64_t elem_per_channel, int relu, float* slots_a, float* slots_b,
+                              float* slots_out, void* stream) {
+    if (int st = validate(n, num_channel, elem_per_channel, "bias_add_act_stats")) return st;
+    if (!a || !bias_a || !b || !out) { set_error("bias_add_act_stats: null pointer"); return PPQHIP_ERR_INVALID_VALUE; }
+    if (!bias_b && slots_b) { set_error("bias_add_act_stats: without bias_b, b is only read: it has no sink"); return PPQHIP_ERR_INVALID_VALUE; }
+    EpArgs p{};
+    p.a = a; p.bias_a = bias_a; p.b = b; p.bias_b = bias_b; p.out = out;
+    const bool aligned = aligned16(a) && aligned16(b) && aligned16(out);
+    const EpSinks sk{{slots_a, slots_b, slots_out}};
+    hipStream_t s = (hipStream_t)stream;
+    if (bias_b) return launch_epilogue_stats<true, true>(p, n, num_channel, elem_per_channel, relu, aligned, sk, "bias_add_act_stats", s);
+    return launch_epilogue_stats<true, false>(p, n, num_channel, elem_per_channel, relu, aligned, sk, "bias_add_act_stats", s);
+}
+
+}
diff --git a/ppq_amd/csrc/minmax_fold.hpp b/ppq_amd/csrc/minmax_fold.hpp
--- /dev/null
+++ b/ppq_amd/csrc/minmax_fold.hpp
@@ -0,0 +1,32 @@
+#pragma once
+
+#include "common.hpp"
+
+namespace ppqhip {
+
+__device__ __forceinline__ void minmax_fold1(float& mn, float& mx, float a) {
+    mn = fminf(mn, a);
+    mx = fmaxf(mx, a);
+}
+
+__device__ __forceinline__ void minmax_fold4(float& mn, float& mx, const float4& v) {
+    mn = fminf(fminf(mn, v.x), fminf(v.y, fminf(v.z, v.w)));
+    mx = fmaxf(fmaxf(mx, v.x), fmaxf(v.y, fmaxf(v.z, v.w)));
+}
+
+__device__ __forceinline__ void minmax_block_fold(float& mn, float& mx, float* lds) {
+    mn = wave_min(mn);
+    mx = wave_max(mx);
+    const int wid = threadIdx.x >> 6, lane = threadIdx.x & 63, nw = blockDim.x >> 6;
+    if (lane == 0) { lds[wid] = mn; lds[16 + wid] = mx; }
+    __syncthreads();
+    if (threadIdx.x == 0)
+        for (int w = 1; w < nw; w++) { mn = fminf(mn, lds[w]); mx = fmaxf(mx, lds[16 + w]); }
+}
+
+__device__ __forceinline__ void minmax_slot_fold(float* slot, float mn, float mx) {
+    slot[0] = fminf(mn, slot[0]);
+    slot[1] = fmaxf(mx, slot[1]);
+}
+
+}
diff --git a/ppq_amd/csrc/reduce.hip b/ppq_amd/csrc/reduce.hip
--- a/ppq_amd/csrc/reduce.hip
+++ b/ppq_amd/csrc/reduce.hip
@@ -3,6 +3,7 @@
 #include <vector>
 
 #include "common.hpp"
+#include "minmax_fold.hpp"
 
 namespace ppqhip {
 
@@ -25,17 +26,12 @@
 __global__ __launch_bounds__(kBlock) void minmax_t_kernel(const float* __restrict__ x, uint32_t n, int vec_ok,
                                                           float* __restrict__ minmax, float* __restrict__ partial,
                                                           int accumulate) {
-    __shared__ float lds[16];
+    __shared__ float lds[32];
     float mn = INFINITY, mx = -INFINITY;
-    stream_elems<U, NT>(x, n, vec_ok != 0, [&](float a) { mn = fminf(mn, a); mx = fmaxf(mx, a); });
+    stream_elems<U, NT>(x, n, vec_ok != 0, [&](float a) { minmax_fold1(mn, mx, a); });
     if (partial == nullptr) { block_minmax_commit(mn, mx, &minmax[0], &minmax[1], lds); return; }
-    mn = wave_min(mn);
-    mx = wave_max(mx);
-    const int wid = threadIdx.x >> 6, lane = threadIdx.x & 63;
-    if (lane == 0) { lds[wid] = mn; lds[8 + wid] = mx; }
-    __syncthreads();
+    minmax_block_fold(mn, mx, lds);
     if (threadIdx.x == 0) {
-        for (int w = 1; w < kBlock / kWave; w++) { mn = fminf(mn, lds[w]); mx = fmaxf(mx, lds[8 + w]); }
         if (accumulate) {
             mn = fminf(mn, partial[2 * blockIdx.x]);
             mx = fmaxf(mx, partial[2 * blockIdx.x + 1]);
@@ -102,10 +98,7 @@
             };
             auto consume = [&](const float4 (&buf)[kMMU]) {
 #pragma unroll
-                for (int u = 0; u < kMMU; u++) {
-                    mn = fminf(fminf(mn, buf[u].x), fminf(buf[u].y, fminf(buf[u].z, buf[u].w)));
-                    mx = fmaxf(fmaxf(mx, buf[u].x), fmaxf(buf[u].y, fmaxf(buf[u].z, buf[u].w)));
-                }
+                for (int u = 0; u < kMMU; u++) minmax_fold4(mn, mx, buf[u]);
             };
             fetch(bufa, k);
             for (;;) {
@@ -122,19 +115,11 @@
 #pragma unroll 4
             for (int r = 0; r < 4 * kMMU; r++) {
                 const uint32_t i = e0 + r * kMMBlock;
-                if (i < n) { const float a = x[i]; mn = fminf(mn, a); mx = fmaxf(mx, a); }
+                if (i < n) minmax_fold1(mn, mx, x[i]);
             }
         }
-        mn = wave_min(mn);
-        mx = wave_max(mx);
-        const int wid = threadIdx.x >> 6, lane = threadIdx.x & 63;
-        if (lane == 0) { lds[wid] = mn; lds[16 + wid] = mx; }
-        __syncthreads();
-        if (threadIdx.x == 0) {
-            for (int w = 1; w < kMMBlock / kWave; w++) { mn = fminf(mn, lds[w]); mx = fmaxf(mx, lds[16 + w]); }
-            job.slots[2 * g] = fminf(mn, job.slots[2 * g]);
-            job.slots[2 * g + 1] = fmaxf(mx, job.slots[2 * g + 1]);
-        }
+        minmax_block_fold(mn, mx, lds);
+        if (threadIdx.x == 0) minmax_slot_fold(job.slots + 2 * g, mn, mx);
         __syncthreads();
     }
 }
@@ -156,10 +141,7 @@
     };
     auto fold = [&](const float4 (&buf)[K]) {
 #pragma unroll
-        for (int k = 0; k < K; k++) {
-            mn = fminf(fminf(mn, buf[k].x), fminf(buf[k].y, fminf(buf[k].z, buf[k].w)));
-            mx = fmaxf(fmaxf(mx, buf[k].x), fmaxf(buf[k].y, fmaxf(buf[k].z, buf[k].w)));
-        }
+        for (int k = 0; k < K; k++) minmax_fold4(mn, mx, buf[k]);
     };
     if (PING) {
         if (r0 < r1) {
@@ -185,15 +167,10 @@
         }
     }
     if (g == G - 1) {
-        for (uint32_t i = full_rows * kMMBlock * 4 + threadIdx.x; i < n; i += kMMBlock) { const float a = x[i]; mn = fminf(mn, a); mx = fmaxf(mx, a); }
-    }
-    mn = wave_min(mn);
-    mx = wave_max(mx);
-    const int wid = threadIdx.x >> 6, lane = threadIdx.x & 63;
-    if (lane == 0) { lds[wid] = mn; lds[16 + wid] = mx; }
-    __syncthreads();
+        for (uint32_t i = full_rows * kMMBlock * 4 + threadIdx.x; i < n; i += kMMBlock) minmax_fold1(mn, mx, x[i]);
+    }
+    minmax_block_fold(mn, mx, lds);
     if (threadIdx.x == 0) {
-        for (int w = 1; w < kMMBlock / kWave; w++) { mn = fminf(mn, lds[w]); mx = fmaxf(mx, lds[16 + w]); }
         slots[2 * g] = fminf(mn, s_mn);
         slots[2 * g + 1] = fmaxf(mx, s_mx);
     }
@@ -201,22 +178,14 @@
 
 __global__ __launch_bounds__(kBlock) void minmax_finish_kernel(const float* __restrict__ partial, uint32_t count,
                                                                float* __restrict__ minmax) {
-    __shared__ float lds[16];
+    __shared__ float lds[32];
     float mn = INFINITY, mx = -INFINITY;
     for (uint32_t i = threadIdx.x; i < count; i += kBlock) {
         mn = fminf(mn, partial[2 * i]);
         mx = fmaxf(mx, partial[2 * i + 1]);
     }
-    mn = wave_min(mn);
-    mx = wave_max(mx);
-    const int wid = threadIdx.x >> 6, lane = threadIdx.x & 63;
-    if (lane == 0) { lds[wid] = mn; lds[8 + wid] = mx; }
-    __syncthreads();
-    if (threadIdx.x == 0) {
-        for (int w = 1; w < kBlock / kWave; w++) { mn = fminf(mn, lds[w]); mx = fmaxf(mx, lds[8 + w]); }
-        minmax[0] = fminf(minmax[0], mn);
-        minmax[1] = fmaxf(minmax[1], mx);
-    }
+    minmax_block_fold(mn, mx, lds);
+    if (threadIdx.x == 0) minmax_slot_fold(minmax, mn, mx);
 }
 
 constexpr int kMMCU = 16;
diff --git a/ppq_amd/ffi.py b/ppq_amd/ffi.py
--- a/ppq_amd/ffi.py
+++ b/ppq_amd/ffi.py
@@ -184,6 +184,45 @@
         _raise(lib.ppqhip_bias_add_act(a.data_ptr(), bias_a.data_ptr(), b.data_ptr(), 0 if bias_b is None else bias_b.data_ptr(),
                                        out.data_ptr(), a.numel(), geo[0], geo[1], 1 if relu else 0, _stream()))
     return out
+
+
+def _sink_slots(job, dev) -> int:
+    if job is None: return 0
+    slots = job[1]
+    if (job[0] != 'minmax' or slots.dtype is not _F32 or slots.device != dev or not slots.is_contiguous()
+            or slots.numel() != 2 * lib.ppqhip_minmax_slots()): raise ValueError('no sink for this job')
+    return slots.data_ptr()
+
+
+def _fused_or_raise(status: int) -> bool:
+    if status == _lib.NOT_FUSED: return False
+    _raise(status)
+    return True
+
+
+def bias_act_stats_(y: torch.Tensor, bias: torch.Tensor, relu: bool, job) -> bool:
+    geo = _epilogue_geometry([y], [bias])
+    if geo is None or job is None: return False
+    try: slots = _sink_slots(job, y.device)
+    except ValueError: return False
+    with _DeviceOf(y):
+        return _fused_or_raise(lib.ppqhip_bias_act_stats(y.data_ptr(), bias.data_ptr(), y.numel(), geo[0], geo[1],
+                                                         1 if relu else 0, slots, _stream()))
+
+
+def bias_add_act_stats(a: torch.Tensor, bias_a: torch.Tensor, b: torch.Tensor, bias_b, relu: bool, job_a, job_b, job_out):
+    geo = _epilogue_geometry([a, b], [bias_a] if bias_b is None else [bias_a, bias_b])
+    if geo is None or a.data_ptr() == b.data_ptr(): return None
+    if bias_b is None and job_b is not None: return None
+    try: slots = [_sink_slots(j, a.device) for j in (job_a, job_b, job_out)]
+    except ValueError: return None
+    if not any(slots): return None
+    out = torch.empty_like(a)
+    with _DeviceOf(a):
+        ok = _fused_or_raise(lib.ppqhip_bias_add_act_stats(
+            a.data_ptr(), bias_a.data_ptr(), b.data_ptr(), 0 if bias_b is None else bias_b.data_ptr(), out.data_ptr(),
+            a.numel(), geo[0], geo[1], 1 if relu else 0, slots[0], slots[1], slots[2], _stream()))
+    return out if ok else None
 
 
 _ADAROUND_JOB = np.dtype([('w', '<u8'), ('v', '<u8'), ('scale', '<u8'), ('offset', '<u8'), ('out', '<u8'), ('dy', '<u8'),
diff --git a/ppq_amd/harness.py b/ppq_amd/harness.py
--- a/ppq_amd/harness.py
+++ b/ppq_amd/harness.py
@@ -401,7 +401,7 @@
         return plan
 
     def _run_epilogue(self, grp: EpilogueGroup, raw_of: Callable, hooks) -> Optional[Dict[str, torch.Tensor]]:
-        from .ffi import bias_act_, bias_add_act
+        from .ffi import bias_act_, bias_act_stats_, bias_add_act, bias_add_act_stats
         for conv in grp.convs:
             x, w = raw_of(conv.inputs[0]), conv.inputs[1].value
             if not (isinstance(x, torch.Tensor) and x.is_cuda and x.dtype == torch.float32 and x.dim() == 4
@@ -432,7 +432,10 @@
         if grp.kind == 'P1':
             conv = grp.convs[0]
             y = ys[conv.name]
-            if not bias_act_(y, biases[conv.name], relu=True):
+            stored = {grp.relu.name: y}
+            fed = self._epilogue_sinks(grp, hooks, stored, y)
+            if fed is not None and not bias_act_stats_(y, biases[conv.name], True, fed[0].get(grp.relu.name)): fed = None
+            if fed is None and not bias_act_(y, biases[conv.name], relu=True):
                 y.add_(biases[conv.name].view(1, -1, 1, 1)).relu_()
             tail = {conv.name: y, grp.relu.name: y}
         else:
@@ -440,13 +443,25 @@
             a = ys[conv_a.name]
             conv_b = grp.convs[1] if len(grp.convs) > 1 else None
             b = ys[conv_b.name] if conv_b is not None else raw_of(grp.add.inputs[1])
-            out = bias_add_act(a, biases[conv_a.name], b, biases[conv_b.name] if conv_b is not None else None, relu=True)
+            bias_b = biases[conv_b.name] if conv_b is not None else None
+            stored = {conv_a.name: a, grp.relu.name: None}
+            if conv_b is not None: stored[conv_b.name] = b
+            fed, out = self._epilogue_sinks(grp, hooks, stored, a), None
+            if fed is not None:
+                jobs = fed[0]
+                out = bias_add_act_stats(a, biases[conv_a.name], b, bias_b, True, jobs.get(conv_a.name),
+                                         jobs.get(conv_b.name) if conv_b is not None else None, jobs.get(grp.relu.name))
+                if out is None: fed = None
+                else: stored[grp.relu.name] = out
+            if out is None: out = bias_add_act(a, biases[conv_a.name], b, bias_b, relu=True)
             if out is None:
                 a.add_(biases[conv_a.name].view(1, -1, 1, 1))
                 if conv_b is not None: b.add_(biases[conv_b.name].view(1, -1, 1, 1))
                 out = F.relu(a + b)
             tail = {conv_a.name: a, grp.add.name: out, grp.relu.name: out}
             if conv_b is not None: tail[conv_b.name] = b
+        if fed is not None:
+            for name, job in fed[0].items(): fed[1].prepay(stored[name], job[1])
         values: Dict[str, torch.Tensor] = {}
         for op in grp.ops:
             hook = hooks.get(op.name)
@@ -467,6 +482,22 @@
                 outs = hook.post_forward_hook(outputs=fp_outs, quant_outputs=outs, quant_configs=out_cfgs)
             for v, y in zip(op.outputs, outs): values[v.name] = y
         return values
+
+    @ staticmethod
+    def _epilogue_sinks(grp: EpilogueGroup, hooks, stored: Dict[str, torch.Tensor], like: torch.Tensor):
+        jobs, queue = {}, None
+        for op in grp.ops:
+            hook = hooks.get(op.name)
+            if hook is None or not isinstance(op, QuantableOperation): continue
+            for cfg in op.config.output_quantization_config:
+                ob = hook._observer_table.get(cfg)
+                if ob is None: continue
+                if op.name not in stored or op.name in jobs or hook.stream is not None or ob.queue is None: return None
+                if queue is not None and ob.queue is not queue: return None
+                job = ob.stat_job(like)
+                if job is None: return None
+                jobs[op.name], queue = job, ob.queue
+        return (jobs, queue) if jobs else None
 
     def _quantize_parameter(self, var: Variable, config) -> torch.Tensor:
         hit = self._fused.get((var.name, id(config)))
diff --git a/ppq_amd/observer.py b/ppq_amd/observer.py
--- a/ppq_amd/observer.py
+++ b/ppq_amd/observer.py
@@ -104,6 +104,7 @@
         self._max = max_pending_bytes
         self.launches = 0
         self.recorder: Optional[list] = None
+        self._prepaid = set()
 
     def __len__(self):
         return (len(self._minmax) + len(self._minmax_c) + sum(len(v) for v in self._hist.values())
@@ -111,14 +112,24 @@
 
     def _grow(self, value) -> None:
         self._bytes += value.numel() * 4
-        if self._bytes > self._max: self.flush()
+        if self._bytes > self._max: self._launch()
+
+    def prepay(self, value: torch.Tensor, buffer: torch.Tensor) -> None:
+        self._prepaid.add((value.data_ptr(), buffer.data_ptr()))
+
+    def _claim(self, value: torch.Tensor, buffer: torch.Tensor) -> bool:
+        key = (value.data_ptr(), buffer.data_ptr())
+        if key not in self._prepaid: return False
+        self._prepaid.discard(key)
+        return True
 
     def add_minmax(self, value: torch.Tensor, slots: torch.Tensor) -> None:
+        if self._prepaid and self._claim(value, slots): return
         self._minmax.append((value, slots))
         self._grow(value)
 
     def add_minmax_c(self, value: torch.Tensor, channel_axis: int, mins: torch.Tensor, maxs: torch.Tensor, fresh: bool) -> None:
-        if any(m.data_ptr() == mins.data_ptr() for _, _, m, _, _ in self._minmax_c): self.flush()
+        if any(m.data_ptr() == mins.data_ptr() for _, _, m, _, _ in self._minmax_c): self._launch()
         self._minmax_c.append((value, channel_axis, mins, maxs, bool(fresh)))
         self._grow(value)
 
@@ -133,6 +144,10 @@
         return dest
 
     def flush(self) -> None:
+        self._prepaid.clear()
+        self._launch()
+
+    def _launch(self) -> None:
         if self._quantile:
             pending, self._quantile = self._quantile, {}
             for (q, _), items in pending.items():
@@ -206,6 +221,9 @@
     def observe(self, value):
         raise NotImplementedError('Implement this function first.')
 
+    def stat_job(self, value) -> Optional[tuple]:
+        return None
+
     def render_quantization_config(self):
         raise NotImplementedError('Implement this function first.')
 
@@ -261,12 +279,9 @@
         if not is_initial(self._quant_cfg): return
         cfg = self._quant_cfg
         if cfg.policy.has_property(P.PER_TENSOR):
-            if self._range is None:
-                seed = _range_seed(value.device)
-                self._range = seed[0].clone()
-                self._slots = seed[1].clone()
-            if self.queue is not None and value.is_cuda: self.queue.add_minmax(value, self._slots)
-            else: CUDA.MinMax_T_Slots(value, self._slots)
+            _, slots = TorchMinMaxObserver.stat_job(self, value)
+            if self.queue is not None and value.is_cuda: self.queue.add_minmax(value, slots)
+            else: CUDA.MinMax_T_Slots(value, slots)
             self._slots_dirty = True
         elif cfg.policy.has_property(P.PER_CHANNEL):
             queued = (self.queue is not None and value.is_cuda and CUDA.minmax_c_outer_is_one(value, cfg.channel_axis))
@@ -284,6 +299,15 @@
             raise TypeError('Min-max Observer only work with per-tensor or per-channel quantize policy.')
         self._observed = True
         self._host_range = None
+
+    def stat_job(self, value: torch.Tensor) -> Optional[tuple]:
+        cfg = self._quant_cfg
+        if not is_initial(cfg) or not cfg.policy.has_property(P.PER_TENSOR): return None
+        if self._range is None:
+            seed = _range_seed(value.device)
+            self._range = seed[0].clone()
+            self._slots = seed[1].clone()
+        return ('minmax', self._slots)
 
     def _fold(self) -> None:
         if self._queued_c:
@@ -384,6 +408,9 @@
                     CUDA.Histogram_T(tensor=value, histogram=self._hist, scale=self._hist_scale)
             else:
                 raise TypeError('Quantization Property is invalid, expect either ASYMMETRICAL or SYMMETRICAL config here.')
+
+    def stat_job(self, value: torch.Tensor) -> Optional[tuple]:
+        return super().stat_job(value) if self._phase == 'Detecting Minmax' else None
 
     def pending_range(self):
         return super().pending_range() if self._phase == 'Detecting Minmax' else None
```
